# 0xPARC/plonky2-aes

Measured on AMD Instinct MI355X. Metric: proofs/sec (AES-GCM 1 KiB circuit), higher is better.
Workload: dtype u64 (Goldilocks field)

## Files before the change

### bindings/plonky2-hip/src/ffi.rs

```rust
#![allow(non_camel_case_types, dead_code)]
use std::os::raw::{c_char, c_int, c_long, c_void};

#[repr(C)] pub struct P2Builder { _private: [u8; 0] }
#[repr(C)] pub struct P2Circuit { _private: [u8; 0] }
#[repr(C)] pub struct P2Assignment { pub targets: *const u64, pub values: *const u64, pub count: usize }
#[repr(C)] #[derive(Default, Clone, Copy)]
pub struct P2CircuitInfo {
    pub degree_bits: u32, pub num_wires: u32, pub num_routed_wires: u32, pub num_constants_cols: u32, pub num_zs_cols: u32,
    pub num_quotient_cols: u32, pub num_luts: u32, pub num_ops: u32, pub num_levels: u32, pub num_slots: u32,
    pub num_virtual_targets: u32, pub num_fri_rounds: u32, pub proof_bytes: u64, pub zero_knowledge: u32, pub num_gate_kinds: u32,
    pub num_public_inputs: u32, pub hasher: u32,
}
#[repr(C)] pub struct P2KernelTime { pub name: [c_char; 48], pub ms: f32, pub count: u32 }
#[repr(C)] #[derive(Default, Clone, Copy, Debug)]
pub struct P2WitnessFault { pub kind: i32, pub op_kind: i32, pub input_index: i64, pub target: u64, pub gate_row: u32, pub computed: u64, pub found: u64 }

pub const P2_OK: c_int = 0;
pub const P2_PROOF_OK: c_int = 0;
pub const P2_VALUE_UNSET: u64 = u64::MAX;
pub const P2_FAULT_KINDS: [&str; 6] = ["NONE", "INPUT_NOT_CANONICAL", "INPUT_CONFLICT", "LOOKUP_MISS", "GENERATOR_CONFLICT", "NOT_SET"];
pub const P2_HASHER_POSEIDON: c_int = 0;
pub const P2_HASHER_KECCAK: c_int = 1;
pub const P2_POINT_WORDS: usize = 10;
pub const P2_SCALAR_LIMBS: usize = 5;
// ... 24 lines not shown
    pub fn p2_builder_split_le(a0: *mut P2Builder, x: u64, num_bits: usize, bits: *mut u64) -> c_int;
    pub fn p2_builder_range_check(a0: *mut P2Builder, x: u64, num_bits: usize) -> c_int;
    pub fn p2_builder_le_bytes_sum(a0: *mut P2Builder, bytes: *const u64, n: usize, out: *mut u64) -> c_int;
    pub fn p2_builder_split_bytes_le(a0: *mut P2Builder, x: u64, num_bytes: usize, u8_table_idx: usize, bytes: *mut u64) -> c_int;
    pub fn p2_builder_is_less_than(a0: *mut P2Builder, x: u64, y: u64, num_bits: usize, out: *mut u64) -> c_int;
    pub fn p2_builder_register_public_input(a0: *mut P2Builder, t: u64) -> c_int;
    pub fn p2_builder_add_lookup_table_from_pairs(a0: *mut P2Builder, pairs: *const u16, n_pairs: usize) -> usize;
    pub fn p2_builder_add_lookup_from_index(a0: *mut P2Builder, looking_in: u64, lut_index: usize) -> u64;
    pub fn p2_builder_num_gates(a0: *const P2Builder) -> usize;
    pub fn p2_builder_build(a0: *mut P2Builder, blob: *mut *mut u8, blob_len: *mut usize) -> c_int;
    pub fn p2_blob_free(blob: *mut u8);
    pub fn p2_aes_sbox_lut(a0: *mut P2Builder) -> usize;
    pub fn p2_aes_byte_xor_lut(a0: *mut P2Builder) -> usize;
    pub fn p2_aes_gf_2_8_mul_lut(a0: *mut P2Builder) -> usize;
    pub fn p2_gcm_u8_unit_right_shift_lut(a0: *mut P2Builder) -> usize;
    pub fn p2_gcm_u8_bitref_lut(a0: *mut P2Builder) -> usize;
    pub fn p2_gcm_clmul_lo_lut(a0: *mut P2Builder) -> usize;
    pub fn p2_gcm_clmul_hi_lut(a0: *mut P2Builder) -> usize;
    pub fn p2_aes_add_virtual_byte_target(a0: *mut P2Builder, u8_table_idx: usize) -> u64;
    pub fn p2_aes_add_virtual_byte_target_unsafe(a0: *mut P2Builder) -> u64;
    pub fn p2_aes_state_sub_bytes(a0: *mut P2Builder, sbox_lut: usize, s: *const u64, out: *mut u64);
    pub fn p2_aes_state_mix_columns(a0: *mut P2Builder, xor_lut: usize, mul_lut: usize, s: *const u64, out: *mut u64);
    pub fn p2_aes_gf_2_8_mul(a0: *mut P2Builder, mul_lut: usize, x: u64, y: u64) -> u64;
    pub fn p2_aes_gf_2_8_add(a0: *mut P2Builder, xor_lut: usize, x: u64, y: u64) -> u64;
    pub fn p2_aes_key_expansion(a0: *mut P2Builder, nk: c_int, nr: c_int, xor_lut: usize, sbox_lut: usize, key: *const u64, out: *mut u64);
    pub fn p2_aes_encrypt_block(a0: *mut P2Builder, nr: c_int, xor_lut: usize, mul_lut: usize, sbox_lut: usize, state: *const u64, expanded_key: *const u64, out_state: *mut u64);
    pub fn p2_gcm_gctr(a0: *mut P2Builder, nr: c_int, xor_lut: usize, mul_lut: usize, sbox_lut: usize, expanded_key: *const u64, icb: *const u64, x: *const u64, len: usize, y: *mut u64);
    pub fn p2_gcm_right_shift_one(a0: *mut P2Builder, shift_lut: usize, v: *const u64, out: *mut u64);
    pub fn p2_gcm_inc32(a0: *mut P2Builder, block: *const u64, out: *mut u64);
    pub fn p2_gcm_gf_2_128_mul(a0: *mut P2Builder, xor_lut: usize, shift_lut: usize, bitref_lut: usize, x: *const u64, y: *const u64, out: *mut u64);
    pub fn p2_gcm_ghash(a0: *mut P2Builder, xor_lut: usize, shift_lut: usize, bitref_lut: usize, h: *const u64, x: *const u64, len: usize, out: *mut u64) -> c_int;
    pub fn p2_gcm_gf_2_128_mul_tables(a0: *mut P2Builder, xor_lut: usize, clmul_lo_lut: usize, clmul_hi_lut: usize, x: *const u64, y: *const u64, out: *mut u64) -> c_int;
    pub fn p2_gcm_ghash_tables(a0: *mut P2Builder, xor_lut: usize, clmul_lo_lut: usize, clmul_hi_lut: usize, h: *const u64, x: *const u64, len: usize, out: *mut u64, lanes: c_int) -> c_int;
    pub fn p2_builder_set_ghash_tables(a0: *mut P2Builder, lanes: c_int) -> c_int;
    pub fn p2_aes_gcm_build(a0: *mut P2Builder, nk: c_int, nr: c_int, L: usize, with_tag: c_int, key: *mut u64, nonce: *mut u64, pt: *mut u64, ct: *mut u64, tag: *mut u64) -> c_int;
    pub fn p2_builder_hash_n_to_m_no_pad(a0: *mut P2Builder, inputs: *const u64, n: usize, outputs: *mut u64, m: usize) -> c_int;
    pub fn p2_builder_permute_swapped(a0: *mut P2Builder, inputs: *const u64, swap: u64, out: *mut u64) -> c_int;
    pub fn p2_builder_hash_or_noop(a0: *mut P2Builder, inputs: *const u64, n: usize, out: *mut u64) -> c_int;
    pub fn p2_builder_add_virtual_hash(a0: *mut P2Builder, out: *mut u64) -> c_int;
    pub fn p2_builder_add_virtual_cap(a0: *mut P2Builder, cap_height: c_int, out: *mut u64) -> c_int;
    pub fn p2_builder_connect_hashes(a0: *mut P2Builder, x: *const u64, y: *const u64) -> c_int;
    pub fn p2_builder_verify_merkle_proof_to_cap(a0: *mut P2Builder, leaf: *const u64, leaf_len: usize, index_bits: *const u64, n_bits: usize, cap: *const u64, cap_height: c_int, siblings: *const u64, n_siblings: usize) -> c_int;
    pub fn p2_builder_verify_merkle_proof(a0: *mut P2Builder, leaf: *const u64, leaf_len: usize, index_bits: *const u64, n_bits: usize, root: *const u64, siblings: *const u64, n_siblings: usize) -> c_int;
    pub fn p2_native_merkle_cap(leaves: *const u64, num_leaves: usize, leaf_len: usize, cap_height: c_int, cap: *mut u64) -> c_int;
    pub fn p2_native_merkle_prove(leaves: *const u64, num_leaves: usize, leaf_len: usize, cap_height: c_int, index: usize, siblings: *mut u64) -> c_int;
    pub fn p2_native_merkle_verify(leaf: *const u64, leaf_len: usize, index: usize, siblings: *const u64, depth: usize, cap: *const u64, cap_height: c_int, status: *mut c_int) -> c_int;
    pub fn p2_poseidon_cipher_build(a0: *mut P2Builder, L: usize, ks: *mut u64, m: *mut u64, nonce: *mut u64, ct: *mut u64) -> c_int;
    pub fn p2_native_hash_n_to_m_no_pad(in: *const u64, n: usize, out: *mut u64, m: usize);
    pub fn p2_native_poseidon_encrypt(ks10: *const u64, msg: *const u64, n_msg: usize, nonce2: *const u64, ct: *mut u64);
    pub fn p2_native_poseidon_decrypt(ks10: *const u64, ct: *const u64, n_ct: usize, nonce2: *const u64, l: usize, msg: *mut u64) -> c_int;
    pub fn p2_ecgfp5_group_order(out: *mut u64);
    pub fn p2_ecgfp5_generator(out: *mut u64);
    pub fn p2_ecgfp5_mul(k: *const u64, p: *const u64, out: *mut u64);
    pub fn p2_ecgfp5_add(p: *const u64, q: *const u64, out: *mut u64);
    pub fn p2_ecgfp5_neg(p: *const u64, out: *mut u64);
    pub fn p2_ecgfp5_is_in_subgroup(p: *const u64) -> c_int;
    pub fn p2_ecgfp5_compress(p: *const u64, w: *mut u64);
    pub fn p2_ecgfp5_decompress(w: *const u64, out: *mut u64) -> c_int;
    pub fn p2_ecgfp5_random_scalar(out: *mut u64) -> c_int;
    pub fn p2_ecgfp5_random_point(out: *mut u64) -> c_int;
    pub fn p2_ecgfp5_encode_binary(limbs: *const u32, out: *mut u64) -> c_int;
    pub fn p2_ecgfp5_random_scalar_seeded(seed: u64, out: *mut u64);
    pub fn p2_ecgfp5_random_point_seeded(seed: u64, out: *mut u64);
    pub fn p2_ecgfp5_encode_binary_seeded(limbs: *const u32, seed: u64, out: *mut u64);
    pub fn p2_ecgfp5_decode_binary(p: *const u64, limbs: *mut u32);
    pub fn p2_elgamal_encrypt(pk: *const u64, nonce: *const u64, msg: *const u64, c0: *mut u64, c1: *mut u64) -> c_int;
    pub fn p2_elgamal_decrypt(sk: *const u64, c0: *const u64, c1: *const u64, msg: *mut u64) -> c_int;
    pub fn p2_hashed_elgamal_encrypt(pk: *const u64, nonce: *const u64, msg: *const u64, c0: *mut u64, ct: *mut u64) -> c_int;
    pub fn p2_hashed_elgamal_decrypt(sk: *const u64, c0: *const u64, ct: *const u64, msg: *mut u64) -> c_int;
    pub fn p2_builder_add_virtual_point_target(a0: *mut P2Builder, out: *mut u64);
    pub fn p2_builder_constant_point(a0: *mut P2Builder, p: *const u64, out: *mut u64);
    pub fn p2_builder_add_virtual_biguint320_target(a0: *mut P2Builder, bits: *mut u64);
    pub fn p2_builder_multiply_point(a0: *mut P2Builder, bits: *const u64, p: *const u64, out: *mut u64) -> c_int;
    pub fn p2_builder_add_point(a0: *mut P2Builder, p: *const u64, q: *const u64, out: *mut u64);
    pub fn p2_builder_set_ec_gate(a0: *mut P2Builder, on: c_int) -> c_int;
    pub fn p2_builder_ec_step(a0: *mut P2Builder, acc: *const u64, q: *const u64, bit: u64, hinted: c_int, mid: *mut u64, out: *mut u64) -> c_int;
    pub fn p2_builder_public_key(a0: *mut P2Builder, sk_bits: *const u64, pk: *mut u64) -> c_int;
    pub fn p2_builder_elgamal_encrypt(a0: *mut P2Builder, pk: *const u64, nonce_bits: *const u64, msg: *const u64, c0: *mut u64, c1: *mut u64) -> c_int;
    pub fn p2_builder_hashed_elgamal_encrypt(a0: *mut P2Builder, pk: *const u64, nonce_bits: *const u64, msg: *const u64, c0: *mut u64, ct: *mut u64) -> c_int;
    pub fn p2_selftest_host(seed: u64, n_reductions: usize, n_permutations: usize) -> c_int;
    pub fn p2_selftest_device(seed: u64, threads: usize, device: c_int) -> c_int;
    pub fn p2_selftest_lazy_device(seed: u64, threads: usize, device: c_int) -> c_int;
    pub fn p2_selftest_ntt_device(seed: u64, threads: usize, device: c_int) -> c_int;
    pub fn p2_host_poseidon_known(states: *mut u64, n_perm: usize, kind: c_int, rows: u32, parts: c_int) -> c_int;
    pub fn p2_host_partial_rounds(states: *mut u64, count: usize) -> c_int;
    pub fn p2_host_merged_middle(states: *mut u64, count: usize) -> c_int;
    pub fn p2_host_ecstep_constraints(wires: *const u64, count: usize, out: *mut u64) -> c_int;
    pub fn p2_host_ecstep_constraints_ext(wires: *const u64, count: usize, out: *mut u64) -> c_int;
    pub fn p2_host_hash_leaves(data: *const u64, cols: usize, active_cols: usize, num_leaves: usize, digests: *mut u64) -> c_int;
    pub fn p2_native_gf_2_8_mul(a: u8, b: u8) -> u8;
    pub fn p2_native_aes_key_expansion(key: *const u8, nk: c_int, nr: c_int, out: *mut u8);
    pub fn p2_native_aes_encrypt_block(key: *const u8, nk: c_int, nr: c_int, in16: *const u8, out16: *mut u8);
    pub fn p2_native_gf_2_128_mul(x16: *const u8, y16: *const u8, out16: *mut u8);
    pub fn p2_native_ghash(h16: *const u8, x: *const u8, len: usize, out16: *mut u8);
    pub fn p2_native_gctr(key: *const u8, nk: c_int, nr: c_int, icb16: *const u8, x: *const u8, len: usize, y: *mut u8);
    pub fn p2_native_aes_gcm_encrypt(key: *const u8, nk: c_int, nr: c_int, nonce12: *const u8, pt: *const u8, len: usize, ct: *mut u8, tag16: *mut u8);
    pub fn p2_native_keccak_hash_no_pad(in: *const u64, n: usize, out4: *mut u64);
    pub fn p2_native_keccak_two_to_one(l4: *const u64, r4: *const u64, out4: *mut u64);
    pub fn p2_native_keccak256(data: *const u8, len: usize, out32: *mut u8);
    pub fn p2_blob_info(blob: *const u8, len: usize, out: *mut P2CircuitInfo) -> c_int;
    pub fn p2_witness_schedule_check(blob: *const u8, len: usize, fuse: u32, out: *mut u32) -> c_int;
    pub fn p2_verify(blob: *const u8, blob_len: usize, verifier_data: *const u64, verifier_data_len: usize, proof: *const u8, proof_len: usize) -> c_int;
    pub fn p2_vanishing_terms(blob: *const u8, blob_len: usize, openings: *const u8, len: usize, challenges: *const u64, pi_hash: *const u64, terms: *mut u64, cap: usize, n_terms: *mut usize, sides: *mut u64, verdict: *mut c_int) -> c_int;
    pub fn p2_proof_compress(blob: *const u8, blob_len: usize, verifier_data: *const u64, verifier_data_len: usize, proof: *const u8, proof_len: usize, out: *mut u8, cap: usize, n_written: *mut usize) -> c_int;
    pub fn p2_proof_decompress(blob: *const u8, blob_len: usize, verifier_data: *const u64, verifier_data_len: usize, cproof: *const u8, cproof_len: usize, out: *mut u8, cap: usize, n_written: *mut usize) -> c_int;
    pub fn p2_verify_compressed(blob: *const u8, blob_len: usize, verifier_data: *const u64, verifier_data_len: usize, cproof: *const u8, cproof_len: usize) -> c_int;
    pub fn p2_proof_public_inputs(blob: *const u8, blob_len: usize, proof: *const u8, proof_len: usize, out: *mut u64, cap: usize, n_written: *mut usize) -> c_int;
    pub fn p2_circuit_load(blob: *const u8, len: usize, device: c_int) -> *mut P2Circuit;
    pub fn p2_circuit_free(a0: *mut P2Circuit);
    pub fn p2_circuit_verifier_data(a0: *const P2Circuit, out: *mut u64, cap: usize, n_written: *mut usize) -> c_int;
    pub fn p2_circuit_chunk_proofs(a0: *mut P2Circuit) -> usize;
    pub fn p2_circuit_set_zk_key(a0: *mut P2Circuit, key: *const u64) -> c_int;
    pub fn p2_circuit_set_zk_seed(a0: *mut P2Circuit, seed: u64) -> c_int;
    pub fn p2_circuit_proof_bytes(a0: *const P2Circuit) -> usize;
    pub fn p2_circuit_num_public_inputs(a0: *const P2Circuit) -> usize;
    pub fn p2_circuit_public_inputs(a0: *const P2Circuit, proof: *const u8, proof_len: usize, out: *mut u64, cap: usize, n_written: *mut usize) -> c_int;
    pub fn p2_prove_batch(a0: *mut P2Circuit, batch: usize, inputs: *const P2Assignment, proofs: *mut u8, status: *mut c_int) -> c_int;
    pub fn p2_prove_batch_multi(handles: *const *mut P2Circuit, n_handles: usize, batch: usize, inputs: *const P2Assignment, proofs: *mut u8, status: *mut c_int) -> c_int;
    pub fn p2_prove_batch_device(a0: *mut P2Circuit, batch: usize, targets: *const u64, n_targets: usize, d_values: *const u64, d_proofs: *mut u8, d_status: *mut c_int, stream: *mut c_void) -> c_int;
    pub fn p2_circuit_synchronize(a0: *mut P2Circuit) -> c_int;
    pub fn p2_prove_batch_outputs_device(a0: *mut P2Circuit, batch: usize, targets: *const u64, n_targets: usize, d_values: *const u64, out_targets: *const u64, n_out: usize, d_out: *mut u64, d_proofs: *mut u8, d_status: *mut c_int, stream: *mut c_void) -> c_int;
    pub fn p2_prove_batch_outputs(a0: *mut P2Circuit, batch: usize, inputs: *const P2Assignment, out_targets: *const u64, n_out: usize, out_values: *mut u64, proofs: *mut u8, status: *mut c_int) -> c_int;
    pub fn p2_witness_batch_device(a0: *mut P2Circuit, batch: usize, targets: *const u64, n_targets: usize, d_values: *const u64, out_targets: *const u64, n_out: usize, d_out: *mut u64, d_status: *mut c_int, stream: *mut c_void) -> c_int;
    pub fn p2_witness_batch(a0: *mut P2Circuit, batch: usize, inputs: *const P2Assignment, out_targets: *const u64, n_out: usize, out_values: *mut u64, status: *mut c_int) -> c_int;
    pub fn p2_witness_explain(a0: *mut P2Circuit, input: *const P2Assignment, status: *mut c_int, out: *mut c_void) -> c_int;
    pub fn p2_host_witness(blob: *const u8, len: usize, input: *const P2Assignment, out_targets: *const u64, n_out: usize, out_values: *mut u64, status: *mut c_int, fault: *mut c_void) -> c_int;
    pub fn p2_verify_batch(a0: *mut P2Circuit, batch: usize, proofs: *const u8, verifier_data: *const u64, vd_len: usize, status: *mut c_int) -> c_int;
    pub fn p2_verify_batch_device(a0: *mut P2Circuit, batch: usize, d_proofs: *const u8, verifier_data: *const u64, vd_len: usize, d_status: *mut c_int, stream: *mut c_void) -> c_int;
    pub fn p2_gpu_vanishing_flags(a0: *mut P2Circuit, batch: usize, buffers: *const u8, challenges: *const u64, pi_hashes: *const u64, flags: *mut u32) -> c_int;
    pub fn p2_compress_batch(a0: *mut P2Circuit, batch: usize, proofs: *const u8, verifier_data: *const u64, vd_len: usize, out: *mut u8, lengths: *mut u32, status: *mut c_int) -> c_int;
    pub fn p2_decompress_batch(a0: *mut P2Circuit, batch: usize, cproofs: *const u8, lengths: *const u32, verifier_data: *const u64, vd_len: usize, out: *mut u8, status: *mut c_int) -> c_int;
    pub fn p2_verify_compressed_batch(a0: *mut P2Circuit, batch: usize, cproofs: *const u8, lengths: *const u32, verifier_data: *const u64, vd_len: usize, status: *mut c_int) -> c_int;
    pub fn p2_compress_batch_device(a0: *mut P2Circuit, batch: usize, d_proofs: *const u8, verifier_data: *const u64, vd_len: usize, d_out: *mut u8, d_lengths: *mut u32, d_status: *mut c_int, stream: *mut c_void) -> c_int;
    pub fn p2_decompress_batch_device(a0: *mut P2Circuit, batch: usize, d_cproofs: *const u8, d_lengths: *const u32, verifier_data: *const u64, vd_len: usize, d_out: *mut u8, d_status: *mut c_int, stream: *mut c_void) -> c_int;
    pub fn p2_verify_compressed_batch_device(a0: *mut P2Circuit, batch: usize, d_cproofs: *const u8, d_lengths: *const u32, verifier_data: *const u64, vd_len: usize, d_status: *mut c_int, stream: *mut c_void) -> c_int;
    pub fn p2_circuit_set_option(a0: *mut P2Circuit, name: *const c_char, value: c_long) -> c_int;
    pub fn p2_circuit_set_timing(a0: *mut P2Circuit, enable: c_int) -> c_int;
    pub fn p2_circuit_get_timing(a0: *mut P2Circuit, out: *mut P2KernelTime, cap: usize) -> usize;
    pub fn p2_merkle_tree_new(leaves: *const u64, num_leaves: usize, leaf_len: usize, cap_height: c_int, device: c_int, tree: *mut *mut c_void) -> c_int;
    pub fn p2_merkle_tree_new_device(d_leaves: *const u64, num_leaves: usize, leaf_len: usize, cap_height: c_int, device: c_int, stream: *mut c_void, tree: *mut *mut c_void) -> c_int;
    pub fn p2_merkle_tree_free(tree: *mut c_void);
    pub fn p2_merkle_tree_cap(tree: *mut c_void, cap: *mut u64, cap_words: usize) -> c_int;
    pub fn p2_merkle_tree_prove_batch(tree: *mut c_void, indices: *const u64, n: usize, siblings: *mut u64) -> c_int;
    pub fn p2_merkle_tree_prove_batch_device(tree: *mut c_void, d_indices: *const u64, n: usize, d_out: *mut u64, out_stride_words: usize, d_status: *mut c_int, stream: *mut c_void) -> c_int;
    pub fn p2_merkle_verify_batch(leaves: *const u64, leaf_len: usize, indices: *const u64, siblings: *const u64, depth: usize, cap: *const u64, cap_height: c_int, n: usize, status: *mut c_int, device: c_int) -> c_int;
    pub fn p2_merkle_verify_batch_device(d_leaves: *const u64, leaf_len: usize, d_indices: *const u64, d_siblings: *const u64, depth: usize, d_cap: *const u64, cap_height: c_int, n: usize, d_status: *mut c_int, device: c_int, stream: *mut c_void) -> c_int;
    pub fn p2_gpu_merkle_build_device(d_leaves: *const u64, num_leaves: usize, leaf_len: usize, cap_height: c_int, with_transpose: c_int, d_scratch: *mut u64, d_dig: *mut u64, device: c_int, stream: *mut c_void) -> c_int;
    pub fn p2_gpu_device_count() -> c_int;
    pub fn p2_gpu_poseidon(states: *mut u64, n_perm: usize, device: c_int) -> c_int;
    pub fn p2_gpu_lde(coeffs: *const u64, cols: usize, degree_bits: c_int, rate_bits: c_int, lde: *mut u64, device: c_int) -> c_int;
    pub fn p2_gpu_intt(values: *const u64, cols: usize, degree_bits: c_int, coeffs: *mut u64, device: c_int) -> c_int;
    pub fn p2_gpu_lde_round(coeffs: *const u64, cols: usize, degree_bits: c_int, arities: *const u32, n_rounds: usize, round: usize, batch: usize, in_batch_stride: usize, out: *mut u64, out_batch_stride: usize, device: c_int) -> c_int;
    pub fn p2_gpu_quotient_chunks(qvals: *const u64, chunks: usize, degree_bits: c_int, batch: usize, out: *mut u64, device: c_int) -> c_int;
    pub fn p2_gpu_merkle_cap(cols_major: *const u64, cols: usize, num_leaves: usize, cap_height: c_int, cap: *mut u64, device: c_int) -> c_int;
    pub fn p2_gpu_merkle_cap_hasher(cols_major: *const u64, cols: usize, num_leaves: usize, cap_height: c_int, hasher: c_int, cap: *mut u64, device: c_int) -> c_int;
    pub fn p2_gpu_hash_leaves(data: *const u64, cols: usize, active_cols: usize, num_leaves: usize, batch: usize, digests: *mut u64, device: c_int) -> c_int;
    pub fn p2_gpu_partial_rounds(states: *mut u64, count: usize, device: c_int) -> c_int;
    pub fn p2_gpu_merged_middle(states: *mut u64, count: usize, device: c_int) -> c_int;
    pub fn p2_gpu_ecstep_constraints(wires: *const u64, count: usize, out: *mut u64, device: c_int) -> c_int;
    pub fn p2_gpu_merkle_level(child: *const u64, num_parents: usize, batch: usize, parent: *mut u64, device: c_int) -> c_int;
    pub fn p2_gpu_hash_fri_leaves(vals: *const u64, len: usize, arity: c_int, batch: usize, digests: *mut u64, device: c_int) -> c_int;
    pub fn p2_gpu_zeta_pows(z: *const u64, n: usize, pows: *mut u64, device: c_int) -> c_int;
    pub fn p2_circuit_debug_read(a0: *mut P2Circuit, name: *const c_char, index: usize, out: *mut u64, cap: usize, n_written: *mut usize) -> c_int;
}
```

### include/p2aes.h

```cpp
#ifndef P2AES_H
#define P2AES_H
#include <stddef.h>
#include <stdint.h>

#ifdef __cplusplus
extern "C" {
#endif

enum {
    P2_OK = 0,
    P2_ERR_INVALID = 1,
    P2_ERR_NO_DEVICE = 2,
    P2_ERR_HIP = 3,
    P2_ERR_VERIFY = 4
};
enum {
    P2_PROOF_OK = 0,
    P2_PROOF_WITNESS_CONFLICT = 1,
    P2_PROOF_MISSING_INPUT = 2,
    P2_PROOF_ZETA_IN_SUBGROUP = 3,
    P2_PROOF_POW_NOT_FOUND = 4
};
enum {
    P2_VERIFY_OK = 0,
// ... 55 lines not shown
p2_target p2_aes_add_virtual_byte_target(p2_builder*, size_t u8_table_idx);
p2_target p2_aes_add_virtual_byte_target_unsafe(p2_builder*);
void p2_aes_state_sub_bytes(p2_builder*, size_t sbox_lut, const p2_target* s, p2_target* out);
void p2_aes_state_mix_columns(p2_builder*, size_t xor_lut, size_t mul_lut, const p2_target* s, p2_target* out);
p2_target p2_aes_gf_2_8_mul(p2_builder*, size_t mul_lut, p2_target x, p2_target y);
p2_target p2_aes_gf_2_8_add(p2_builder*, size_t xor_lut, p2_target x, p2_target y);
void p2_aes_key_expansion(p2_builder*, int nk, int nr, size_t xor_lut, size_t sbox_lut, const p2_target* key, p2_target* out);
void p2_aes_encrypt_block(p2_builder*, int nr, size_t xor_lut, size_t mul_lut, size_t sbox_lut, const p2_target* state,
                          const p2_target* expanded_key, p2_target* out_state);
void p2_gcm_gctr(p2_builder*, int nr, size_t xor_lut, size_t mul_lut, size_t sbox_lut, const p2_target* expanded_key,
                 const p2_target* icb, const p2_target* x, size_t len, p2_target* y);
void p2_gcm_right_shift_one(p2_builder*, size_t shift_lut, const p2_target* v, p2_target* out);
void p2_gcm_inc32(p2_builder*, const p2_target* block, p2_target* out);
void p2_gcm_gf_2_128_mul(p2_builder*, size_t xor_lut, size_t shift_lut, size_t bitref_lut, const p2_target* x,
                         const p2_target* y, p2_target* out);
int p2_gcm_ghash(p2_builder*, size_t xor_lut, size_t shift_lut, size_t bitref_lut, const p2_target* h, const p2_target* x,
                 size_t len, p2_target* out);
int p2_gcm_gf_2_128_mul_tables(p2_builder*, size_t xor_lut, size_t clmul_lo_lut, size_t clmul_hi_lut, const p2_target* x,
                               const p2_target* y, p2_target* out);
int p2_gcm_ghash_tables(p2_builder*, size_t xor_lut, size_t clmul_lo_lut, size_t clmul_hi_lut, const p2_target* h,
                        const p2_target* x, size_t len, p2_target* out, int lanes);
int p2_builder_set_ghash_tables(p2_builder*, int lanes);
int p2_aes_gcm_build(p2_builder*, int nk, int nr, size_t L, int with_tag, p2_target* key, p2_target* nonce, p2_target* pt,
                     p2_target* ct, p2_target* tag);

int p2_builder_hash_n_to_m_no_pad(p2_builder*, const p2_target* inputs, size_t n, p2_target* outputs, size_t m);
int p2_builder_permute_swapped(p2_builder*, const p2_target inputs[12], p2_target swap, p2_target out[12]);
int p2_builder_hash_or_noop(p2_builder*, const p2_target* inputs, size_t n, p2_target out[4]);
int p2_builder_add_virtual_hash(p2_builder*, p2_target out[4]);
int p2_builder_add_virtual_cap(p2_builder*, int cap_height, p2_target* out);
int p2_builder_connect_hashes(p2_builder*, const p2_target x[4], const p2_target y[4]);
int p2_builder_verify_merkle_proof_to_cap(p2_builder*, const p2_target* leaf, size_t leaf_len, const p2_target* index_bits, size_t n_bits,
                                          const p2_target* cap, int cap_height, const p2_target* siblings, size_t n_siblings);
int p2_builder_verify_merkle_proof(p2_builder*, const p2_target* leaf, size_t leaf_len, const p2_target* index_bits, size_t n_bits,
                                   const p2_target root[4], const p2_target* siblings, size_t n_siblings);
int p2_native_merkle_cap(const uint64_t* leaves, size_t num_leaves, size_t leaf_len, int cap_height, uint64_t* cap);
int p2_native_merkle_prove(const uint64_t* leaves, size_t num_leaves, size_t leaf_len, int cap_height, size_t index, uint64_t* siblings);
int p2_native_merkle_verify(const uint64_t* leaf, size_t leaf_len, size_t index, const uint64_t* siblings, size_t depth, const uint64_t* cap,
                            int cap_height, int* status);
int p2_poseidon_cipher_build(p2_builder*, size_t L, p2_target* ks, p2_target* m, p2_target* nonce, p2_target* ct);
void p2_native_hash_n_to_m_no_pad(const uint64_t* in, size_t n, uint64_t* out, size_t m);
void p2_native_poseidon_encrypt(const uint64_t* ks10, const uint64_t* msg, size_t n_msg, const uint64_t* nonce2, uint64_t* ct);
int p2_native_poseidon_decrypt(const uint64_t* ks10, const uint64_t* ct, size_t n_ct, const uint64_t* nonce2, size_t l, uint64_t* msg);

#define P2_POINT_WORDS 10
#define P2_SCALAR_LIMBS 5
#define P2_SCALAR_BITS 320
void p2_ecgfp5_group_order(uint64_t out[5]);
void p2_ecgfp5_generator(uint64_t out[10]);
void p2_ecgfp5_mul(const uint64_t k[5], const uint64_t p[10], uint64_t out[10]);
void p2_ecgfp5_add(const uint64_t p[10], const uint64_t q[10], uint64_t out[10]);
void p2_ecgfp5_neg(const uint64_t p[10], uint64_t out[10]);
int p2_ecgfp5_is_in_subgroup(const uint64_t p[10]);
void p2_ecgfp5_compress(const uint64_t p[10], uint64_t w[5]);
int p2_ecgfp5_decompress(const uint64_t w[5], uint64_t out[10]);
int p2_ecgfp5_random_scalar(uint64_t out[5]);
int p2_ecgfp5_random_point(uint64_t out[10]);
int p2_ecgfp5_encode_binary(const uint32_t limbs[5], uint64_t out[10]);
void p2_ecgfp5_random_scalar_seeded(uint64_t seed, uint64_t out[5]);
void p2_ecgfp5_random_point_seeded(uint64_t seed, uint64_t out[10]);
void p2_ecgfp5_encode_binary_seeded(const uint32_t limbs[5], uint64_t seed, uint64_t out[10]);
void p2_ecgfp5_decode_binary(const uint64_t p[10], uint32_t limbs[5]);
int p2_elgamal_encrypt(const uint64_t pk[10], const uint64_t nonce[5], const uint64_t msg[10], uint64_t c0[10], uint64_t c1[10]);
int p2_elgamal_decrypt(const uint64_t sk[5], const uint64_t c0[10], const uint64_t c1[10], uint64_t msg[10]);
int p2_hashed_elgamal_encrypt(const uint64_t pk[10], const uint64_t nonce[5], const uint64_t msg[5], uint64_t c0[10], uint64_t ct[5]);
int p2_hashed_elgamal_decrypt(const uint64_t sk[5], const uint64_t c0[10], const uint64_t ct[5], uint64_t msg[5]);
void p2_builder_add_virtual_point_target(p2_builder*, p2_target out[10]);
void p2_builder_constant_point(p2_builder*, const uint64_t p[10], p2_target out[10]);
void p2_builder_add_virtual_biguint320_target(p2_builder*, p2_target bits[320]);
int p2_builder_multiply_point(p2_builder*, const p2_target bits[320], const p2_target p[10], p2_target out[10]);
void p2_builder_add_point(p2_builder*, const p2_target p[10], const p2_target q[10], p2_target out[10]);
int p2_builder_set_ec_gate(p2_builder*, int on);
int p2_builder_ec_step(p2_builder*, const p2_target acc[20], const p2_target q[10], p2_target bit, int hinted, p2_target mid[20], p2_target out[20]);
int p2_builder_public_key(p2_builder*, const p2_target sk_bits[320], p2_target pk[10]);
int p2_builder_elgamal_encrypt(p2_builder*, const p2_target pk[10], const p2_target nonce_bits[320], const p2_target msg[10],
                               p2_target c0[10], p2_target c1[10]);
int p2_builder_hashed_elgamal_encrypt(p2_builder*, const p2_target pk[10], const p2_target nonce_bits[320], const p2_target msg[5],
                                      p2_target c0[10], p2_target ct[5]);

int p2_selftest_host(uint64_t seed, size_t n_reductions, size_t n_permutations);
int p2_selftest_device(uint64_t seed, size_t threads, int device);
int p2_selftest_lazy_device(uint64_t seed, size_t threads, int device);
int p2_selftest_ntt_device(uint64_t seed, size_t threads, int device);
int p2_host_poseidon_known(uint64_t* states, size_t n_perm, int kind, uint32_t rows, int parts);
int p2_host_partial_rounds(uint64_t* states, size_t count);
int p2_host_merged_middle(uint64_t* states, size_t count);
int p2_host_ecstep_constraints(const uint64_t* wires, size_t count, uint64_t* out);
int p2_host_ecstep_constraints_ext(const uint64_t* wires, size_t count, uint64_t* out);
int p2_host_hash_leaves(const uint64_t* data, size_t cols, size_t active_cols, size_t num_leaves, uint64_t* digests);

uint8_t p2_native_gf_2_8_mul(uint8_t a, uint8_t b);
void p2_native_aes_key_expansion(const uint8_t* key, int nk, int nr, uint8_t* out );
void p2_native_aes_encrypt_block(const uint8_t* key, int nk, int nr, const uint8_t* in16, uint8_t* out16);
void p2_native_gf_2_128_mul(const uint8_t* x16, const uint8_t* y16, uint8_t* out16);
void p2_native_ghash(const uint8_t* h16, const uint8_t* x, size_t len, uint8_t* out16);
void p2_native_gctr(const uint8_t* key, int nk, int nr, const uint8_t* icb16, const uint8_t* x, size_t len, uint8_t* y);
void p2_native_aes_gcm_encrypt(const uint8_t* key, int nk, int nr, const uint8_t* nonce12, const uint8_t* pt, size_t len,
                               uint8_t* ct, uint8_t* tag16);

void p2_native_keccak_hash_no_pad(const uint64_t* in, size_t n, uint64_t out4[4]);
void p2_native_keccak_two_to_one(const uint64_t l4[4], const uint64_t r4[4], uint64_t out4[4]);
void p2_native_keccak256(const uint8_t* data, size_t len, uint8_t out32[32]);

typedef struct {
    uint32_t degree_bits, num_wires, num_routed_wires, num_constants_cols, num_zs_cols, num_quotient_cols, num_luts,
        num_ops, num_levels, num_slots, num_virtual_targets, num_fri_rounds;
    uint64_t proof_bytes;
    uint32_t zero_knowledge, num_gate_kinds;
    uint32_t num_public_inputs;
    uint32_t hasher;
} p2_circuit_info;
int p2_blob_info(const uint8_t* blob, size_t len, p2_circuit_info* out);
int p2_witness_schedule_check(const uint8_t* blob, size_t len, uint32_t fuse, uint32_t out[4]);
int p2_verify(const uint8_t* blob, size_t blob_len, const uint64_t* verifier_data, size_t verifier_data_len,
              const uint8_t* proof, size_t proof_len);
int p2_vanishing_terms(const uint8_t* blob, size_t blob_len, const uint8_t* openings, size_t len, const uint64_t challenges[16],
                       const uint64_t pi_hash[4], uint64_t* terms, size_t cap, size_t* n_terms, uint64_t sides[8], int* verdict);
int p2_proof_compress(const uint8_t* blob, size_t blob_len, const uint64_t* verifier_data, size_t verifier_data_len, const uint8_t* proof,
                      size_t proof_len, uint8_t* out, size_t cap, size_t* n_written);
int p2_proof_decompress(const uint8_t* blob, size_t blob_len, const uint64_t* verifier_data, size_t verifier_data_len, const uint8_t* cproof,
                        size_t cproof_len, uint8_t* out, size_t cap, size_t* n_written);
int p2_verify_compressed(const uint8_t* blob, size_t blob_len, const uint64_t* verifier_data, size_t verifier_data_len,
                         const uint8_t* cproof, size_t cproof_len);
int p2_proof_public_inputs(const uint8_t* blob, size_t blob_len, const uint8_t* proof, size_t proof_len, uint64_t* out, size_t cap,
                           size_t* n_written);

typedef struct p2_circuit p2_circuit;
p2_circuit* p2_circuit_load(const uint8_t* blob, size_t len, int device);
void p2_circuit_free(p2_circuit*);
int p2_circuit_verifier_data(const p2_circuit*, uint64_t* out, size_t cap, size_t* n_written);
size_t p2_circuit_chunk_proofs(p2_circuit*);
int p2_circuit_set_zk_key(p2_circuit*, const uint64_t key[4]);
int p2_circuit_set_zk_seed(p2_circuit*, uint64_t seed);
size_t p2_circuit_proof_bytes(const p2_circuit*);
size_t p2_circuit_num_public_inputs(const p2_circuit*);
int p2_circuit_public_inputs(const p2_circuit*, const uint8_t* proof, size_t proof_len, uint64_t* out, size_t cap, size_t* n_written);
typedef struct {
    const p2_target* targets;
    const uint64_t* values;
    size_t count;
} p2_assignment;
int p2_prove_batch(p2_circuit*, size_t batch, const p2_assignment* inputs, uint8_t* proofs, int* status);
int p2_prove_batch_multi(p2_circuit* const* handles, size_t n_handles, size_t batch, const p2_assignment* inputs,
                         uint8_t* proofs, int* status);
int p2_prove_batch_device(p2_circuit*, size_t batch, const p2_target* targets, size_t n_targets, const uint64_t* d_values,
                          uint8_t* d_proofs, int* d_status, void* stream);
int p2_circuit_synchronize(p2_circuit*);

#define P2_VALUE_UNSET UINT64_MAX
int p2_prove_batch_outputs_device(p2_circuit*, size_t batch, const p2_target* targets, size_t n_targets, const uint64_t* d_values,
                                  const p2_target* out_targets, size_t n_out, uint64_t* d_out, uint8_t* d_proofs, int* d_status, void* stream);
int p2_prove_batch_outputs(p2_circuit*, size_t batch, const p2_assignment* inputs, const p2_target* out_targets, size_t n_out,
                           uint64_t* out_values, uint8_t* proofs, int* status);
int p2_witness_batch_device(p2_circuit*, size_t batch, const p2_target* targets, size_t n_targets, const uint64_t* d_values,
                            const p2_target* out_targets, size_t n_out, uint64_t* d_out, int* d_status, void* stream);
int p2_witness_batch(p2_circuit*, size_t batch, const p2_assignment* inputs, const p2_target* out_targets, size_t n_out,
                     uint64_t* out_values, int* status);
typedef struct {
    int32_t kind;
    int32_t op_kind;
    int64_t input_index;
    p2_target target;
    uint32_t gate_row;
    uint64_t computed, found;
} p2_witness_fault;
enum {
// ... 75 lines not shown
```

### plonky2-aes_amd/api.py

```python
import ctypes as C
import os
import struct

P = 0xFFFFFFFF00000001


class P2Error(RuntimeError):
    pass


class ProveError(P2Error):

    def __init__(self, status):
        self.status = status
        super().__init__({1: "witness conflict or lookup input not in table", 2: "a generator never ran (missing input)",
                          3: "opening point is in the subgroup",
                          4: "no proof-of-work witness found"}.get(status, "prove failed (%d)" % status))


VERIFY_OK, VERIFY_SHAPE, VERIFY_NON_CANONICAL, VERIFY_POW, VERIFY_ZETA_IN_SUBGROUP, VERIFY_VANISHING = 0, 1, 2, 3, 4, 5
VERIFY_MERKLE_INITIAL, VERIFY_FRI_FOLD, VERIFY_MERKLE_FRI, VERIFY_FINAL_POLY = 6, 7, 8, 9
VERIFY_REASONS = {
    "": VERIFY_OK,
    "proof truncated": VERIFY_SHAPE,
# ... 106 lines not shown
    _fields_ = [("name", C.c_char * 48), ("ms", C.c_float), ("count", C.c_uint32)]


def lib():
    global _lib
    if _lib is not None:
        return _lib
    path = lib_path()
    if not os.path.exists(path):
        raise P2Error("native library %s is missing: run `python -c 'import __graft_entry__ as g; g.build()'`" % path)
    L = C.CDLL(path)
    vp = C.c_void_p
    sig = {
        "p2_last_error": (C.c_char_p, []),
        "p2_builder_new": (vp, []), "p2_builder_new_zk": (vp, []), "p2_builder_free": (None, [vp]),
        "p2_builder_new_config": (vp, [C.c_int, C.c_int]), "p2_builder_set_hasher": (C.c_int, [vp, C.c_int]),
        "p2_native_keccak_hash_no_pad": (None, [u64p, sz, u64p]), "p2_native_keccak_two_to_one": (None, [u64p, u64p, u64p]),
        "p2_native_keccak256": (None, [C.c_char_p, sz, C.c_char_p]),
        "p2_gpu_merkle_cap_hasher": (C.c_int, [u64p, sz, sz, C.c_int, C.c_int, u64p, C.c_int]),
        "p2_circuit_set_zk_seed": (C.c_int, [vp, u64]),
        "p2_circuit_set_zk_key": (C.c_int, [vp, C.POINTER(u64)]),
        "p2_circuit_set_option": (C.c_int, [vp, C.c_char_p, C.c_long]),
        "p2_prove_batch_multi": (C.c_int, [C.POINTER(vp), sz, sz, C.POINTER(_Assignment), C.c_char_p, C.POINTER(C.c_int)]),
        "p2_builder_add_virtual_target": (u64, [vp]), "p2_builder_constant": (u64, [vp, u64]),
        "p2_builder_zero": (u64, [vp]), "p2_builder_one": (u64, [vp]),
        "p2_builder_arithmetic": (u64, [vp, u64, u64, u64, u64, u64]),
        "p2_builder_mul_const_add": (u64, [vp, u64, u64, u64]),
        "p2_builder_add": (u64, [vp, u64, u64]), "p2_builder_sub": (u64, [vp, u64, u64]), "p2_builder_mul": (u64, [vp, u64, u64]),
        "p2_builder_select": (u64, [vp, u64, u64, u64]), "p2_builder_is_equal": (u64, [vp, u64, u64]),
        "p2_builder_connect": (None, [vp, u64, u64]),
        "p2_builder_assert_bool": (C.c_int, [vp, u64]), "p2_builder_range_check": (C.c_int, [vp, u64, sz]),
        "p2_builder_le_sum": (C.c_int, [vp, u64p, sz, u64p]), "p2_builder_le_bytes_sum": (C.c_int, [vp, u64p, sz, u64p]),
        "p2_builder_split_le": (C.c_int, [vp, u64, sz, u64p]), "p2_builder_split_bytes_le": (C.c_int, [vp, u64, sz, sz, u64p]),
        "p2_builder_is_less_than": (C.c_int, [vp, u64, u64, sz, u64p]),
        "p2_builder_register_public_input": (C.c_int, [vp, u64]),
        "p2_proof_public_inputs": (C.c_int, [C.c_char_p, sz, C.c_char_p, sz, u64p, sz, C.POINTER(sz)]),
        "p2_builder_add_lookup_table_from_pairs": (sz, [vp, u16p, sz]),
        "p2_builder_add_lookup_from_index": (u64, [vp, u64, sz]),
        "p2_builder_num_gates": (sz, [vp]),
        "p2_builder_build": (C.c_int, [vp, C.POINTER(u8p), C.POINTER(sz)]), "p2_blob_free": (None, [u8p]),
        "p2_aes_sbox_lut": (sz, [vp]), "p2_aes_byte_xor_lut": (sz, [vp]), "p2_aes_gf_2_8_mul_lut": (sz, [vp]),
        "p2_gcm_u8_unit_right_shift_lut": (sz, [vp]), "p2_gcm_u8_bitref_lut": (sz, [vp]),
        "p2_aes_add_virtual_byte_target": (u64, [vp, sz]), "p2_aes_add_virtual_byte_target_unsafe": (u64, [vp]),
        "p2_aes_state_sub_bytes": (None, [vp, sz, u64p, u64p]),
        "p2_aes_state_mix_columns": (None, [vp, sz, sz, u64p, u64p]),
        "p2_aes_gf_2_8_mul": (u64, [vp, sz, u64, u64]), "p2_aes_gf_2_8_add": (u64, [vp, sz, u64, u64]),
        "p2_aes_key_expansion": (None, [vp, C.c_int, C.c_int, sz, sz, u64p, u64p]),
        "p2_aes_encrypt_block": (None, [vp, C.c_int, sz, sz, sz, u64p, u64p, u64p]),
        "p2_gcm_gctr": (None, [vp, C.c_int, sz, sz, sz, u64p, u64p, u64p, sz, u64p]),
        "p2_gcm_right_shift_one": (None, [vp, sz, u64p, u64p]), "p2_gcm_inc32": (None, [vp, u64p, u64p]),
        "p2_gcm_gf_2_128_mul": (None, [vp, sz, sz, sz, u64p, u64p, u64p]),
        "p2_gcm_ghash": (C.c_int, [vp, sz, sz, sz, u64p, u64p, sz, u64p]),
        "p2_gcm_clmul_lo_lut": (sz, [vp]), "p2_gcm_clmul_hi_lut": (sz, [vp]),
        "p2_gcm_gf_2_128_mul_tables": (C.c_int, [vp, sz, sz, sz, u64p, u64p, u64p]),
        "p2_gcm_ghash_tables": (C.c_int, [vp, sz, sz, sz, u64p, u64p, sz, u64p, C.c_int]),
        "p2_builder_set_ghash_tables": (C.c_int, [vp, C.c_int]),
        "p2_aes_gcm_build": (C.c_int, [vp, C.c_int, C.c_int, sz, C.c_int, u64p, u64p, u64p, u64p, u64p]),
        "p2_builder_hash_n_to_m_no_pad": (C.c_int, [vp, u64p, sz, u64p, sz]),
        "p2_poseidon_cipher_build": (C.c_int, [vp, sz, u64p, u64p, u64p, u64p]),
        "p2_native_hash_n_to_m_no_pad": (None, [u64p, sz, u64p, sz]),
        "p2_native_poseidon_encrypt": (None, [u64p, u64p, sz, u64p, u64p]),
        "p2_native_poseidon_decrypt": (C.c_int, [u64p, u64p, sz, u64p, sz, u64p]),
        "p2_ecgfp5_group_order": (None, [u64p]), "p2_ecgfp5_generator": (None, [u64p]),
        "p2_ecgfp5_mul": (None, [u64p, u64p, u64p]), "p2_ecgfp5_add": (None, [u64p, u64p, u64p]), "p2_ecgfp5_neg": (None, [u64p, u64p]),
        "p2_ecgfp5_is_in_subgroup": (C.c_int, [u64p]),
        "p2_ecgfp5_compress": (None, [u64p, u64p]), "p2_ecgfp5_decompress": (C.c_int, [u64p, u64p]),
        "p2_ecgfp5_random_scalar": (C.c_int, [u64p]), "p2_ecgfp5_random_point": (C.c_int, [u64p]),
        "p2_ecgfp5_encode_binary": (C.c_int, [u32p, u64p]),
        "p2_ecgfp5_random_scalar_seeded": (None, [u64, u64p]), "p2_ecgfp5_random_point_seeded": (None, [u64, u64p]),
        "p2_ecgfp5_encode_binary_seeded": (None, [u32p, u64, u64p]), "p2_ecgfp5_decode_binary": (None, [u64p, u32p]),
        "p2_elgamal_encrypt": (C.c_int, [u64p, u64p, u64p, u64p, u64p]), "p2_elgamal_decrypt": (C.c_int, [u64p, u64p, u64p, u64p]),
        "p2_hashed_elgamal_encrypt": (C.c_int, [u64p, u64p, u64p, u64p, u64p]),
        "p2_hashed_elgamal_decrypt": (C.c_int, [u64p, u64p, u64p, u64p]),
        "p2_builder_add_virtual_point_target": (None, [vp, u64p]), "p2_builder_constant_point": (None, [vp, u64p, u64p]),
        "p2_builder_add_virtual_biguint320_target": (None, [vp, u64p]),
        "p2_builder_multiply_point": (C.c_int, [vp, u64p, u64p, u64p]), "p2_builder_add_point": (None, [vp, u64p, u64p, u64p]),
        "p2_builder_public_key": (C.c_int, [vp, u64p, u64p]),
        "p2_builder_set_ec_gate": (C.c_int, [vp, C.c_int]), "p2_builder_ec_step": (C.c_int, [vp, u64p, u64p, u64, C.c_int, u64p, u64p]),
        "p2_builder_elgamal_encrypt": (C.c_int, [vp, u64p, u64p, u64p, u64p, u64p]),
        "p2_builder_hashed_elgamal_encrypt": (C.c_int, [vp, u64p, u64p, u64p, u64p, u64p]),
        "p2_selftest_host": (C.c_int, [u64, sz, sz]), "p2_selftest_device": (C.c_int, [u64, sz, C.c_int]),
        "p2_selftest_lazy_device": (C.c_int, [u64, sz, C.c_int]),
        "p2_selftest_ntt_device": (C.c_int, [u64, sz, C.c_int]),
        "p2_native_gf_2_8_mul": (C.c_uint8, [C.c_uint8, C.c_uint8]),
        "p2_native_aes_key_expansion": (None, [C.c_char_p, C.c_int, C.c_int, C.c_char_p]),
        "p2_native_aes_encrypt_block": (None, [C.c_char_p, C.c_int, C.c_int, C.c_char_p, C.c_char_p]),
        "p2_native_gf_2_128_mul": (None, [C.c_char_p, C.c_char_p, C.c_char_p]),
        "p2_native_ghash": (None, [C.c_char_p, C.c_char_p, sz, C.c_char_p]),
        "p2_native_gctr": (None, [C.c_char_p, C.c_int, C.c_int, C.c_char_p, C.c_char_p, sz, C.c_char_p]),
        "p2_native_aes_gcm_encrypt": (None, [C.c_char_p, C.c_int, C.c_int, C.c_char_p, C.c_char_p, sz, C.c_char_p, C.c_char_p]),
        "p2_blob_info": (C.c_int, [C.c_char_p, sz, C.POINTER(_Info)]),
        "p2_witness_schedule_check": (C.c_int, [C.c_char_p, sz, C.c_uint32, u32p]),
        "p2_verify": (C.c_int, [C.c_char_p, sz, u64p, sz, C.c_char_p, sz]),
        "p2_vanishing_terms": (C.c_int, [C.c_char_p, sz, C.c_char_p, sz, u64p, u64p, u64p, sz, C.POINTER(sz), u64p, C.POINTER(C.c_int)]),
        "p2_gpu_vanishing_flags": (C.c_int, [vp, sz, C.c_char_p, u64p, u64p, u32p]),
        "p2_proof_compress": (C.c_int, [C.c_char_p, sz, u64p, sz, C.c_char_p, sz, C.c_char_p, sz, C.POINTER(sz)]),
        "p2_proof_decompress": (C.c_int, [C.c_char_p, sz, u64p, sz, C.c_char_p, sz, C.c_char_p, sz, C.POINTER(sz)]),
        "p2_verify_compressed": (C.c_int, [C.c_char_p, sz, u64p, sz, C.c_char_p, sz]),
        "p2_circuit_load": (vp, [C.c_char_p, sz, C.c_int]), "p2_circuit_free": (None, [vp]),
        "p2_circuit_verifier_data": (C.c_int, [vp, u64p, sz, C.POINTER(sz)]),
        "p2_circuit_proof_bytes": (sz, [vp]),
        "p2_circuit_num_public_inputs": (sz, [vp]),
        "p2_circuit_public_inputs": (C.c_int, [vp, C.c_char_p, sz, u64p, sz, C.POINTER(sz)]),
        "p2_circuit_chunk_proofs": (sz, [vp]),
        "p2_prove_batch": (C.c_int, [vp, sz, C.POINTER(_Assignment), C.c_char_p, C.POINTER(C.c_int)]),
        "p2_prove_batch_device": (C.c_int, [vp, sz, u64p, sz, vp, vp, vp, vp]),
        "p2_circuit_synchronize": (C.c_int, [vp]),
        "p2_prove_batch_outputs": (C.c_int, [vp, sz, C.POINTER(_Assignment), u64p, sz, u64p, C.c_char_p, C.POINTER(C.c_int)]),
        "p2_prove_batch_outputs_device": (C.c_int, [vp, sz, u64p, sz, vp, u64p, sz, vp, vp, vp, vp]),
        "p2_witness_batch": (C.c_int, [vp, sz, C.POINTER(_Assignment), u64p, sz, u64p, C.POINTER(C.c_int)]),
        "p2_witness_batch_device": (C.c_int, [vp, sz, u64p, sz, vp, u64p, sz, vp, vp, vp]),
        "p2_witness_explain": (C.c_int, [vp, C.POINTER(_Assignment), C.POINTER(C.c_int), vp]),
        "p2_host_witness": (C.c_int, [C.c_char_p, sz, C.POINTER(_Assignment), u64p, sz, u64p, C.POINTER(C.c_int), vp]),
        "p2_verify_batch": (C.c_int, [vp, sz, C.c_char_p, u64p, sz, C.POINTER(C.c_int)]),
        "p2_verify_batch_device": (C.c_int, [vp, sz, vp, u64p, sz, vp, vp]),
        "p2_compress_batch": (C.c_int, [vp, sz, C.c_char_p, u64p, sz, C.c_char_p, u32p, C.POINTER(C.c_int)]),
        "p2_compress_batch_device": (C.c_int, [vp, sz, vp, u64p, sz, vp, vp, vp, vp]),
        "p2_decompress_batch": (C.c_int, [vp, sz, C.c_char_p, u32p, u64p, sz, C.c_char_p, C.POINTER(C.c_int)]),
        "p2_decompress_batch_device": (C.c_int, [vp, sz, vp, vp, u64p, sz, vp, vp, vp]),
        "p2_verify_compressed_batch": (C.c_int, [vp, sz, C.c_char_p, u32p, u64p, sz, C.POINTER(C.c_int)]),
        "p2_verify_compressed_batch_device": (C.c_int, [vp, sz, vp, vp, u64p, sz, vp, vp]),
        "p2_circuit_set_timing": (C.c_int, [vp, C.c_int]),
        "p2_circuit_get_timing": (sz, [vp, C.POINTER(_KernelTime), sz]),
        "p2_gpu_device_count": (C.c_int, []),
        "p2_gpu_poseidon": (C.c_int, [u64p, sz, C.c_int]),
        "p2_host_partial_rounds": (C.c_int, [u64p, sz]),
        "p2_gpu_partial_rounds": (C.c_int, [u64p, sz, C.c_int]),
        "p2_host_merged_middle": (C.c_int, [u64p, sz]),
        "p2_gpu_merged_middle": (C.c_int, [u64p, sz, C.c_int]),
        "p2_host_ecstep_constraints": (C.c_int, [u64p, sz, u64p]), "p2_host_ecstep_constraints_ext": (C.c_int, [u64p, sz, u64p]),
        "p2_gpu_ecstep_constraints": (C.c_int, [u64p, sz, u64p, C.c_int]),
        "p2_gpu_lde": (C.c_int, [u64p, sz, C.c_int, C.c_int, u64p, C.c_int]),
        "p2_gpu_intt": (C.c_int, [u64p, sz, C.c_int, u64p, C.c_int]),
        "p2_gpu_lde_round": (C.c_int, [u64p, sz, C.c_int, u32p, sz, sz, sz, sz, u64p, sz, C.c_int]),
        "p2_gpu_quotient_chunks": (C.c_int, [u64p, sz, C.c_int, sz, u64p, C.c_int]),
        "p2_gpu_merkle_cap": (C.c_int, [u64p, sz, sz, C.c_int, u64p, C.c_int]),
        "p2_gpu_zeta_pows": (C.c_int, [u64p, sz, u64p, C.c_int]),
        "p2_circuit_debug_read": (C.c_int, [vp, C.c_char_p, sz, u64p, sz, C.POINTER(sz)]),
        "p2_builder_permute_swapped": (C.c_int, [vp, u64p, u64, u64p]), "p2_builder_hash_or_noop": (C.c_int, [vp, u64p, sz, u64p]),
        "p2_builder_add_virtual_hash": (C.c_int, [vp, u64p]), "p2_builder_add_virtual_cap": (C.c_int, [vp, C.c_int, u64p]),
        "p2_builder_connect_hashes": (C.c_int, [vp, u64p, u64p]),
        "p2_builder_verify_merkle_proof_to_cap": (C.c_int, [vp, u64p, sz, u64p, sz, u64p, C.c_int, u64p, sz]),
        "p2_builder_verify_merkle_proof": (C.c_int, [vp, u64p, sz, u64p, sz, u64p, u64p, sz]),
        "p2_native_merkle_cap": (C.c_int, [u64p, sz, sz, C.c_int, u64p]),
        "p2_native_merkle_prove": (C.c_int, [u64p, sz, sz, C.c_int, sz, u64p]),
        "p2_native_merkle_verify": (C.c_int, [u64p, sz, sz, u64p, sz, u64p, C.c_int, C.POINTER(C.c_int)]),
        "p2_merkle_tree_new": (C.c_int, [u64p, sz, sz, C.c_int, C.c_int, C.POINTER(vp)]),
        "p2_merkle_tree_new_device": (C.c_int, [vp, sz, sz, C.c_int, C.c_int, vp, C.POINTER(vp)]),
        "p2_merkle_tree_free": (None, [vp]), "p2_merkle_tree_cap": (C.c_int, [vp, u64p, sz]),
        "p2_merkle_tree_prove_batch": (C.c_int, [vp, u64p, sz, u64p]),
        "p2_merkle_tree_prove_batch_device": (C.c_int, [vp, vp, sz, vp, sz, vp, vp]),
        "p2_merkle_verify_batch": (C.c_int, [u64p, sz, u64p, u64p, sz, u64p, C.c_int, sz, C.POINTER(C.c_int), C.c_int]),
        "p2_merkle_verify_batch_device": (C.c_int, [vp, sz, vp, vp, sz, vp, C.c_int, sz, vp, C.c_int, vp]),
        "p2_gpu_merkle_build_device": (C.c_int, [vp, sz, sz, C.c_int, C.c_int, vp, vp, C.c_int, vp]),
    }
    missing = []
    for name, (res, args) in sig.items():
        try:
            f = getattr(L, name)
        except AttributeError:
            missing.append(name)
            continue
        f.restype, f.argtypes = res, args
    L._p2_missing = missing
    L._p2_signatures = sig
    _lib = L
# ... 1047 lines not shown
```

### plonky2-aes_amd/csrc/capi_host.cpp

```cpp
#include <stdlib.h>

#include "../../include/p2aes.h"
#include "aes_gadgets.h"
#include "capi_common.h"
#include "compress.h"
#include "ecgfp5.h"
#include "merkle_host.h"
#include "poseidon_cipher.h"
#include "poseidon_fast.h"
#include "verifier.h"
#include "witness_check.h"
#include "witness_schedule.h"

using namespace p2;

namespace p2 {
thread_local std::string g_last_error;
}

struct p2_builder {
    CircuitBuilder b;
};


// ... 531 lines not shown
        ptt_put(ecgfp5::multiply_point(b->b, bits_at(bits), ptt_at(p)), out);
        return P2_OK;
    } catch (std::exception& e) {
        return set_error(e.what()), P2_ERR_INVALID;
    }
}
void p2_builder_add_point(p2_builder* b, const p2_target p[10], const p2_target q[10], p2_target out[10]) { (void)guarded([&] {    ptt_put(ecgfp5::add_point(b->b, ptt_at(p), ptt_at(q)), out);}); }
int p2_builder_public_key(p2_builder* b, const p2_target sk_bits[320], p2_target pk[10]) {
    try {
        ptt_put(ecgfp5::public_key_target(b->b, bits_at(sk_bits)), pk);
        return P2_OK;
    } catch (std::exception& e) {
        return set_error(e.what()), P2_ERR_INVALID;
    }
}
int p2_builder_elgamal_encrypt(p2_builder* b, const p2_target pk[10], const p2_target nonce_bits[320], const p2_target msg[10], p2_target c0[10],
                               p2_target c1[10]) {
    try {
        ecgfp5::PointTarget a, c;
        ecgfp5::elgamal_encrypt_target(b->b, ptt_at(pk), bits_at(nonce_bits), ptt_at(msg), &a, &c);
        ptt_put(a, c0);
        ptt_put(c, c1);
        return P2_OK;
    } catch (std::exception& e) {
        return set_error(e.what()), P2_ERR_INVALID;
    }
}
int p2_builder_hashed_elgamal_encrypt(p2_builder* b, const p2_target pk[10], const p2_target nonce_bits[320], const p2_target msg[5],
                                      p2_target c0[10], p2_target ct[5]) {
    try {
        ecgfp5::PointTarget a;
        ecgfp5::hashed_elgamal_encrypt_target(b->b, ptt_at(pk), bits_at(nonce_bits), msg, &a, ct);
        ptt_put(a, c0);
        return P2_OK;
    } catch (std::exception& e) {
        return set_error(e.what()), P2_ERR_INVALID;
    }
}

int p2_selftest_host(uint64_t seed, size_t n_reductions, size_t n_permutations) {
    u64 x = seed | 1;
    auto rnd = [&]() {
        x ^= x << 13;
        x ^= x >> 7;
        x ^= x << 17;
        return x;
    };
    size_t bad = 0;
    for (size_t i = 0; i < n_reductions; i++) {
        u64 hi = rnd(), lo = rnd();
        switch (i & 15) {
            case 0: hi &= gl::EPS; break;
            case 1: lo &= gl::EPS; break;
            case 2: hi |= ~gl::EPS; break;
            case 3: lo |= ~gl::EPS; break;
            case 4: hi = 0; break;
            case 5: lo = 0; break;
            case 6: hi = ~0ull; lo = ~0ull - (x & 3); break;
            case 7: hi &= ~gl::EPS; lo &= gl::EPS; break;
            default: break;
        }
        unsigned __int128 v = ((unsigned __int128)hi << 64) | lo;
        u64 want = (u64)(v % gl::P);
        if (glf::canon(glf::red128(hi, lo)) != want) bad++;
        if (gl::reduce128(hi, lo) != want) bad++;
        glf::Acc a;
        a.init();
        a.fma(hi, lo);
        a.fma(lo, lo);
        unsigned __int128 w = ((unsigned __int128)hi * lo) % gl::P + ((unsigned __int128)lo * lo) % gl::P;
        if (glf::canon(a.reduce()) != (u64)(w % gl::P)) bad++;
    }
    for (size_t i = 0; i < n_permutations; i++) {
        u64 s0[12], s1[12];
        for (int k = 0; k < 12; k++) s0[k] = s1[k] = (i & 3) == 3 ? rnd() : rnd() % gl::P;
        for (int k = 0; k < 12; k++) s0[k] %= gl::P;
        gl::poseidon(s0);
        glf::poseidon(s1);
        for (int k = 0; k < 12; k++) bad += s0[k] != s1[k];
    }
    return (int)std::min<size_t>(bad, 0x7FFFFFFF);
}

int p2_host_poseidon_known(uint64_t* states, size_t n_perm, int kind, uint32_t rows, int parts) {
    if (kind < 0 || kind > (int)glf::FR_ZERO_RATE || rows == 0 || rows > glf::ROWS_ALL) return set_error("kind must be 0..2 and rows a mask of words 0..11"), P2_ERR_INVALID;
    for (size_t i = 0; i < n_perm; i++) {
        u64* s = states + 12 * i;
        if (parts) {
            glf::first_round_any(s, (u32)kind);
            glf::middle(s);
            glf::last_round_any(s, rows);
        } else {
            glf::permute_known_any(s, (u32)kind, rows);
        }
    }
    return P2_OK;
}
int p2_host_partial_rounds(uint64_t* states, size_t count) {
    for (size_t i = 0; i < count; i++) glf::partial_block(states + 12 * i);
    return P2_OK;
}
int p2_host_merged_middle(uint64_t* states, size_t count) {
    for (size_t i = 0; i < count; i++) glf::merged_middle(states + 12 * i);
    return P2_OK;
}
int p2_host_ecstep_constraints(const uint64_t* wires, size_t count, uint64_t* out) {
    if (count && (!wires || !out)) return set_error("p2_host_ecstep_constraints: null argument"), P2_ERR_INVALID;
    for (size_t i = 0; i < 80 * count; i++)
        if (wires[i] >= gl::P) return set_error("p2_host_ecstep_constraints: non-canonical wire"), P2_ERR_INVALID;
    for (size_t r = 0; r < count; r++)
        ecstep_gate_constraints<FBase>([&](u32 i) { return wires[80 * r + i]; }, [&](int k, u64 c) { out[40 * r + k] = c; });
    return P2_OK;
}
int p2_host_ecstep_constraints_ext(const uint64_t* wires, size_t count, uint64_t* out) {
    if (count && (!wires || !out)) return set_error("p2_host_ecstep_constraints_ext: null argument"), P2_ERR_INVALID;
    for (size_t i = 0; i < 160 * count; i++)
        if (wires[i] >= gl::P) return set_error("p2_host_ecstep_constraints_ext: non-canonical wire"), P2_ERR_INVALID;
    for (size_t r = 0; r < count; r++)
        ecstep_gate_constraints<FExt>([&](u32 i) { return gl::e2(wires[160 * r + 2 * i], wires[160 * r + 2 * i + 1]); },
                                      [&](int k, gl::E2 c) { out[80 * r + 2 * k] = c.a, out[80 * r + 2 * k + 1] = c.b; });
    return P2_OK;
}
int p2_host_hash_leaves(const uint64_t* data, size_t cols, size_t active_cols, size_t num_leaves, uint64_t* digests) {
    if (cols == 0 || cols > (1u << 20)) return set_error("cols out of range"), P2_ERR_INVALID;
    for (size_t leaf = 0; leaf < num_leaves; leaf++) {
        u64 st[12] = {0};
        u64* out = digests + 4 * leaf;
        if (cols <= 4) {
            for (size_t c = 0; c < 4; c++) out[c] = (c < cols && c < active_cols) ? data[c * num_leaves + leaf] : 0;
            continue;
        }
        for (size_t c0 = 0; c0 < cols; c0 += 8) {
            for (size_t k = 0; k < 8 && c0 + k < cols; k++) st[k] = c0 + k < active_cols ? data[(c0 + k) * num_leaves + leaf] : 0;
            glf::sponge_permute(st, (int)c0, (int)cols, (int)std::min(active_cols, cols));
        }
        for (int i = 0; i < 4; i++) out[i] = st[i];
    }
    return P2_OK;
}

uint8_t p2_native_gf_2_8_mul(uint8_t a, uint8_t b) { return aes::gf_2_8_mul(a, b); }
void p2_native_aes_key_expansion(const uint8_t* key, int nk, int nr, uint8_t* out) {
    (void)guarded([&] {
        auto w = aes::key_expansion(nk, nr, key);
        for (size_t i = 0; i < w.size(); i++) memcpy(out + 4 * i, w[i].data(), 4);
    });
}
void p2_native_aes_encrypt_block(const uint8_t* key, int nk, int nr, const uint8_t* in, uint8_t* out) {
    (void)guarded([&] {
        auto w = aes::key_expansion(nk, nr, key);
        auto s = aes::flatten_state(aes::encrypt_block(nr, in, w));
        memcpy(out, s.data(), 16);
    });
}
void p2_native_gf_2_128_mul(const uint8_t* x, const uint8_t* y, uint8_t* out) {
    (void)guarded([&] {
        auto r = aes::gf_2_128_mul(x, y);
        memcpy(out, r.data(), 16);
    });
}
void p2_native_ghash(const uint8_t* h, const uint8_t* x, size_t len, uint8_t* out) {
    (void)guarded([&] {
        auto r = aes::ghash(h, x, len);
        memcpy(out, r.data(), 16);
    });
}
// ... 331 lines not shown
```

### plonky2-aes_amd/csrc/gl.h

```cpp
#pragma once
#include <stdint.h>

#if defined(__HIPCC__)
#include <hip/hip_runtime.h>
#define GL_HD __host__ __device__ __forceinline__
#define GL_D __device__ __forceinline__
#else
#define GL_HD inline
#define GL_D inline
#endif

namespace gl {

typedef uint64_t u64;
typedef uint32_t u32;

static const u64 P = 0xFFFFFFFF00000001ULL;
static const u64 EPS = 0xFFFFFFFFULL;
static const u64 MULT_GEN = 14293326489335486720ULL;
static const u64 POW2_GEN = 7277203076849721926ULL;
static const u64 W_EXT = 7;

#if defined(__HIP_DEVICE_COMPILE__)
typedef unsigned long long sg;
// ... 22 lines not shown
    sg dead;
    asm("v_mad_u64_u32 %0, %1, %2, %3, %4" : "=v"(r), "=s"(dead) : "v"(x), "n"(K), "s"(acc_uniform));
    return r;
}
template <u32 K>
GL_D u64 madk0(u32 x) {
    static_assert(K <= 64, "not an inline constant");
    u64 r;
    sg dead;
    asm("v_mad_u64_u32 %0, %1, %2, %3, 0" : "=v"(r), "=s"(dead) : "v"(x), "n"(K));
    return r;
}
GL_D u64 mad_eps_co(u32 a, u64 c, sg& k) {
    u64 r;
    asm("v_mad_u64_u32 %0, %1, %2, -1, %3" : "=v"(r), "=s"(k) : "v"(a), "v"(c));
    return r;
}
GL_D u64 add_u32(u64 c, u32 x) {
    u64 r;
    sg dead;
    asm("v_mad_u64_u32 %0, %1, %2, 1, %3" : "=v"(r), "=s"(dead) : "v"(x), "v"(c));
    return r;
}
GL_D u64 add_eps_co(u64 c, sg& k) {
    u64 r;
    asm("v_mad_u64_u32 %0, %1, 1, -1, %2" : "=v"(r), "=s"(k) : "v"(c));
    return r;
}
GL_D u32 add_co(u32 x, u32 y, sg& cout) {
    u32 r;
    asm("v_add_co_u32_e64 %0, %1, %2, %3" : "=v"(r), "=s"(cout) : "v"(x), "v"(y));
    return r;
}
GL_D u32 addc_co(u32 x, u32 y, sg cin, sg& cout) {
    u32 r;
    asm("s_nop 1\n\tv_addc_co_u32_e64 %0, %1, %2, %3, %4" : "=v"(r), "=s"(cout) : "v"(x), "v"(y), "s"(cin));
    return r;
}
GL_D u32 sub_co(u32 x, u32 y, sg& cout) {
    u32 r;
    asm("v_sub_co_u32_e64 %0, %1, %2, %3" : "=v"(r), "=s"(cout) : "v"(x), "v"(y));
    return r;
}
GL_D u32 subb_co(u32 x, u32 y, sg cin, sg& cout) {
    u32 r;
    asm("s_nop 1\n\tv_subb_co_u32_e64 %0, %1, %2, %3, %4" : "=v"(r), "=s"(cout) : "v"(x), "v"(y), "s"(cin));
    return r;
}
GL_D u32 subb_co_settled(u32 x, u32 y, sg cin, sg& cout) {
    u32 r;
    asm("v_subb_co_u32_e64 %0, %1, %2, %3, %4" : "=v"(r), "=s"(cout) : "v"(x), "v"(y), "s"(cin));
    return r;
}
GL_D u64 add_eps_where_settled(sg C, u64 Rs) {
    u64 out;
    u32 c01;
    sg dead;
    asm("v_cndmask_b32_e64 %[c], 0, 1, %[m]\n\t"
        "v_mad_u64_u32 %[o], %[d], %[c], -1, %[r]"
        : [o] "=&v"(out), [c] "=&v"(c01), [d] "=&s"(dead)
        : [m] "s"(C), [r] "v"(Rs));
    return out;
}
GL_D u32 subb0_co(u32 x, sg cin, sg& cout) {
    u32 r;
    asm("s_nop 1\n\tv_subb_co_u32_e64 %0, %1, %2, 0, %3" : "=v"(r), "=s"(cout) : "v"(x), "s"(cin));
    return r;
}
GL_D u32 ones_where(sg m) {
    u32 r;
    asm("s_nop 1\n\tv_cndmask_b32_e64 %0, 0, -1, %1" : "=v"(r) : "s"(m));
    return r;
}
GL_D u32 pick(sg m, u32 yes, u32 no) {
    u32 r;
    asm("s_nop 1\n\tv_cndmask_b32_e64 %0, %1, %2, %3" : "=v"(r) : "v"(no), "v"(yes), "s"(m));
    return r;
}
GL_D u32 one_where(sg m) {
    u32 r;
    asm("s_nop 1\n\tv_cndmask_b32_e64 %0, 0, 1, %1" : "=v"(r) : "s"(m));
    return r;
}
template <bool BRANCH = true>
GL_D u64 red_fix(u64 Rs, sg C, sg B) {
    if (!BRANCH) {
        const u32 dh = ones_where(B & ~C);
        const u32 dl = ones_where(C & ~B) - dh;
        u64 d = ((u64)dh << 32) | dl;
        asm("" : "+v"(d));
        return Rs + d;
    }
    sg Cm = C;
    if (__builtin_expect(B != 0, 0)) {
        const u32 dh = ones_where(B & ~C);
        u64 d = ((u64)dh << 32) | (0u - dh);
        asm("" : "+v"(d));
        Rs += d;
        Cm = C & ~B;
    }
    return add_eps_where_settled(Cm, Rs);
}
GL_D u64 pick64(sg m, u64 yes, u64 no) {
    u32 lo, hi;
    asm("s_nop 1\n\tv_cndmask_b32_e64 %0, %3, %2, %6\n\tv_cndmask_b32_e64 %1, %5, %4, %6"
        : "=&v"(lo), "=&v"(hi)
        : "v"((u32)yes), "v"((u32)no), "v"((u32)(yes >> 32)), "v"((u32)(no >> 32)), "s"(m));
    return ((u64)hi << 32) | lo;
}
GL_D u64 pick64_salu(sg m, u64 yes, u64 no) {
    u32 lo, hi;
    asm("v_cndmask_b32_e64 %0, %3, %2, %6\n\tv_cndmask_b32_e64 %1, %5, %4, %6"
        : "=&v"(lo), "=&v"(hi)
        : "v"((u32)yes), "v"((u32)no), "v"((u32)(yes >> 32)), "v"((u32)(no >> 32)), "s"(m));
    return ((u64)hi << 32) | lo;
}
template <bool HAS_ADDEND, bool A_UNIFORM = false, bool BRANCH = true>
GL_D u64 mulr_add_dev(u64 a, u64 b, u64 c) {
    const u32 a0 = (u32)a, a1 = (u32)(a >> 32), b0 = (u32)b, b1 = (u32)(b >> 32);
    const u64 P = HAS_ADDEND ? (u64)a0 * b0 + (u32)c : (u64)a0 * b0;
    u64 Y = (u64)a0 * b1 + (P >> 32);
    if (HAS_ADDEND) Y = add_u32(Y, (u32)(c >> 32));
    sg k, C, b1_, B;
    Y = A_UNIFORM ? mad_co_k(a1, b0, Y, k) : mad_co(a1, b0, Y, k);
    const u64 H = (u64)a1 * b1 + (Y >> 32);
    const u64 lo = (Y << 32) | (u32)P;
    const u64 R = mad_eps_co((u32)H, lo, C);
    const u32 r0 = subb_co_settled((u32)R, (u32)(H >> 32), k, b1_);
    const u32 r1 = subb0_co((u32)(R >> 32), b1_, B);
    return red_fix<BRANCH>(((u64)r1 << 32) | r0, C, B);
}
GL_D u64 red128_dev(u64 hi, u64 lo) {
    sg C, b1_, B;
    const u64 R = mad_eps_co((u32)hi, lo, C);
    const u32 r0 = sub_co((u32)R, (u32)(hi >> 32), b1_);
    const u32 r1 = subb0_co((u32)(R >> 32), b1_, B);
    return red_fix(((u64)r1 << 32) | r0, C, B);
}
GL_D u64 canon_dev(u64 r) {
    sg c;
    const u64 t = add_eps_co(r, c);
    return pick64(c, t, r);
}
#endif

GL_HD u64 add(u64 a, u64 b) {
#if defined(__HIP_DEVICE_COMPILE__)
    sg k, c1, c2;
    const u32 s0 = add_co((u32)a, (u32)b, k);
    const u32 s1 = addc_co((u32)(a >> 32), (u32)(b >> 32), k, c1);
    const u64 t = add_eps_co(((u64)s1 << 32) | s0, c2);
    const sg m = c1 | c2;
    return pick64_salu(m, t, ((u64)s1 << 32) | s0);
#else
    u64 s = a + b;
    if (s < a || s >= P) s -= P;
    return s;
#endif
}
GL_HD u64 add_ref(u64 a, u64 b) {
    u64 s = a + b;
    if (s < a || s >= P) s -= P;
    return s;
}
GL_HD u64 sub(u64 a, u64 b) {
#if defined(__HIP_DEVICE_COMPILE__)
    sg b0, B;
    const u32 d0 = sub_co((u32)a, (u32)b, b0);
    const u32 d1 = subb_co((u32)(a >> 32), (u32)(b >> 32), b0, B);
    const u32 e = ones_where(B);
    u64 fix = ((u64)e << 32) | (0u - e);
    asm("" : "+v"(fix));
    return (((u64)d1 << 32) | d0) + fix;
#else
    return a >= b ? a - b : a + (P - b);
#endif
}
GL_HD u64 sub_ref(u64 a, u64 b) { return a >= b ? a - b : a + (P - b); }
GL_HD u64 neg(u64 a) { return a ? P - a : 0; }
GL_HD u64 dbl(u64 a) { return add(a, a); }

GL_HD void mul64(u64 a, u64 b, u64& hi, u64& lo) {
#if defined(__HIP_DEVICE_COMPILE__)
    lo = a * b;
    hi = __umul64hi(a, b);
#else
    unsigned __int128 m = (unsigned __int128)a * b;
    lo = (u64)m;
    hi = (u64)(m >> 64);
#endif
}

GL_HD u64 reduce128(u64 hi, u64 lo) {
    u64 hi_hi = hi >> 32, hi_lo = hi & EPS;
    u64 t0 = lo - hi_hi;
    if (lo < hi_hi) t0 -= EPS;
    u64 t1 = hi_lo * EPS;
    u64 r = t0 + t1;
    if (r < t1) r += EPS;
    if (r >= P) r -= P;
    return r;
}
GL_HD u64 mul_ref(u64 a, u64 b) {
    u64 hi, lo;
    mul64(a, b, hi, lo);
    return reduce128(hi, lo);
}
GL_HD u64 mul(u64 a, u64 b) {
#if defined(__HIP_DEVICE_COMPILE__)
    return canon_dev(mulr_add_dev<false>(a, b, 0));
#else
    return mul_ref(a, b);
#endif
}
GL_HD u64 mul_nb(u64 a, u64 b) {
#if defined(__HIP_DEVICE_COMPILE__)
    return canon_dev(mulr_add_dev<false, false, false>(a, b, 0));
#else
    return mul_ref(a, b);
#endif
}
GL_HD u64 sqr(u64 a) { return mul(a, a); }
GL_HD u64 mul_add(u64 a, u64 b, u64 c) {
#if defined(__HIP_DEVICE_COMPILE__)
    return canon_dev(mulr_add_dev<true>(a, b, c));
#else
    return add(mul(a, b), c);
#endif
}

GL_HD u64 mul_add_nc(u64 a, u64 b, u64 c) {
#if defined(__HIP_DEVICE_COMPILE__)
    return mulr_add_dev<true>(a, b, c);
#else
    return add(mul(a, b), c);
#endif
}
GL_HD u64 mul_nc(u64 a, u64 b) {
#if defined(__HIP_DEVICE_COMPILE__)
    return mulr_add_dev<false>(a, b, 0);
#else
    return mul(a, b);
#endif
}
GL_HD u64 mul_add_nc_k(u64 k, u64 b, u64 c) {
#if defined(__HIP_DEVICE_COMPILE__)
    return mulr_add_dev<true, true>(k, b, c);
#else
    return add(mul(k, b), c);
#endif
}
GL_HD u64 mul_nc_k(u64 k, u64 b) {
#if defined(__HIP_DEVICE_COMPILE__)
    return mulr_add_dev<false, true>(k, b, 0);
#else
    return mul(k, b);
#endif
}

GL_HD u64 pow(u64 b, u64 e) {
    u64 r = 1;
    while (e) {
        if (e & 1) r = mul(r, b);
        b = sqr(b);
        e >>= 1;
    }
    return r;
}
GL_HD u64 exp_pow2(u64 b, int k) {
    for (int i = 0; i < k; i++) b = sqr(b);
    return b;
}
GL_HD u64 inv(u64 a) { return pow(a, P - 2); }

GL_HD u64 root_of_unity(int k) { return exp_pow2(POW2_GEN, 32 - k); }

GL_HD u32 bitrev(u32 x, int bits) {
    u32 r = 0;
    for (int i = 0; i < bits; i++) {
        r = (r << 1) | (x & 1);
        x >>= 1;
    }
    return r;
}

struct E2 {
    u64 a, b;
};
GL_HD E2 e2(u64 a, u64 b = 0) {
    E2 r;
    r.a = a;
    r.b = b;
    return r;
}
GL_HD E2 add(E2 x, E2 y) { return e2(add(x.a, y.a), add(x.b, y.b)); }
GL_HD E2 sub(E2 x, E2 y) { return e2(sub(x.a, y.a), sub(x.b, y.b)); }
GL_HD E2 mul(E2 x, E2 y) {
    u64 a0b0 = mul(x.a, y.a), a1b1 = mul(x.b, y.b);
    u64 c0 = add(a0b0, mul(a1b1, W_EXT));
    u64 c1 = add(mul(x.a, y.b), mul(x.b, y.a));
    return e2(c0, c1);
}
GL_HD E2 mul(E2 x, u64 s) { return e2(mul(x.a, s), mul(x.b, s)); }
GL_HD E2 sqr(E2 x) { return mul(x, x); }
// ... 103 lines not shown
```

### plonky2-aes_amd/csrc/kernels.h

```cpp
#pragma once
#include <hip/hip_runtime.h>

#include "circuit.h"
#include "witness_schedule.h"
#include "gl.h"
#include "poseidon_fast.h"
#include "poseidon_gate.h"
#include "ecstep_gate.h"
#include "zk_prf.h"

namespace p2k {
using gl::E2;
using gl::u32;
using gl::u64;

static const u64 UNSET = ~0ull;

#ifndef P2_HASH_WAVES_PER_EU
#define P2_HASH_WAVES_PER_EU 5
#endif
#define P2_HASH_WAVES __attribute__((amdgpu_waves_per_eu(P2_HASH_WAVES_PER_EU, P2_HASH_WAVES_PER_EU)))

__global__ __launch_bounds__(256) P2_HASH_WAVES void k_hash_leaves(const u64* __restrict__ data, int cols, int active_cols, size_t col_stride,
                                                      size_t batch_stride, size_t num_leaves, u64* __restrict__ digests,
                                                      size_t dig_batch_stride) {
    if ((size_t)blockIdx.x * blockDim.x + threadIdx.x >= num_leaves) return;
    const u64* d = data + (size_t)blockIdx.y * batch_stride + ((size_t)blockIdx.x * blockDim.x + threadIdx.x);
    u64 st[12];
#pragma unroll
    for (int i = 0; i < 12; i++) st[i] = 0;
    if (cols <= 4) {
        u64* out = digests + (size_t)blockIdx.y * dig_batch_stride + ((size_t)blockIdx.x * blockDim.x + threadIdx.x) * 4;
        for (int c = 0; c < 4; c++) out[c] = (c < cols && c < active_cols) ? d[(size_t)c * col_stride] : 0;
        return;
    }
    for (int c0 = 0; c0 < cols; c0 += 8) {
#pragma unroll
        for (int k = 0; k < 8; k++) {
            int c = c0 + k;
            if (c < cols) st[k] = c < active_cols ? d[(size_t)k * col_stride] : 0;
        }
        d += 8 * col_stride;
        glf::sponge_permute(st, c0, cols, active_cols);
    }
    u64* out = digests + (size_t)blockIdx.y * dig_batch_stride + ((size_t)blockIdx.x * blockDim.x + threadIdx.x) * 4;
#pragma unroll
    for (int i = 0; i < 4; i++) out[i] = st[i];
}

__global__ __launch_bounds__(256) P2_HASH_WAVES void k_hash_fri_leaves(const u64* __restrict__ vals, size_t len, size_t batch_stride, int arity,
                                                          u64* __restrict__ digests, size_t dig_batch_stride) {
    size_t leaf = (size_t)blockIdx.x * blockDim.x + threadIdx.x;
    size_t num_leaves = len / arity;
    if (leaf >= num_leaves) return;
    const u64* v = vals + (size_t)blockIdx.y * batch_stride;
    u64 st[12];
#pragma unroll
    for (int i = 0; i < 12; i++) st[i] = 0;
    int width = 2 * arity;
    for (int e0 = 0; e0 < width; e0 += 8) {
#pragma unroll
        for (int k = 0; k < 8; k++) {
            int e = e0 + k;
            if (e < width) st[k] = v[(size_t)(e & 1) * len + leaf * arity + (e >> 1)];
        }
        glf::sponge_permute(st, e0, width, width);
    }
    u64* out = digests + (size_t)blockIdx.y * dig_batch_stride + leaf * 4;
#pragma unroll
    for (int i = 0; i < 4; i++) out[i] = st[i];
}

__global__ __launch_bounds__(256) P2_HASH_WAVES void k_merkle_level(const u64* __restrict__ child, u64* __restrict__ parent, size_t num_parents,
                                                       size_t batch_stride) {
    if ((size_t)blockIdx.x * blockDim.x + threadIdx.x >= num_parents) return;
    u64 st[12];
    {
        const u64* c = child + (size_t)blockIdx.y * batch_stride + 8 * ((size_t)blockIdx.x * blockDim.x + threadIdx.x);
#pragma unroll
        for (int k = 0; k < 8; k++) st[k] = c[k];
    }
#pragma unroll
    for (int k = 8; k < 12; k++) st[k] = 0;
    glf::two_to_one_permute(st);
    u64* o = parent + (size_t)blockIdx.y * batch_stride + 4 * ((size_t)blockIdx.x * blockDim.x + threadIdx.x);
#pragma unroll
    for (int k = 0; k < 4; k++) o[k] = st[k];
}

__global__ __launch_bounds__(256) P2_HASH_WAVES void k_merkle_top(u64* __restrict__ dig, size_t batch_stride, u32 bits, u32 first_level, u32 num_levels) {
    u64* base = dig + (size_t)blockIdx.y * batch_stride;
    u32 P = ((1u << bits) >> (first_level + 1)) / gridDim.x;
    for (u32 k = 0, l = first_level; k < num_levels; k++, l++, P >>= 1) {
        if (threadIdx.x < P) {
            const size_t off_c = 4 * (((size_t)2 << bits) - ((size_t)2 << (bits - l))), off_p = 4 * (((size_t)2 << bits) - ((size_t)2 << (bits - l - 1)));
            const size_t idx = (size_t)blockIdx.x * P + threadIdx.x;
            u64 st[12];
            {
                const u64* c = base + off_c + 8 * idx;
#pragma unroll
                for (int q = 0; q < 8; q++) st[q] = c[q];
            }
#pragma unroll
            for (int q = 8; q < 12; q++) st[q] = 0;
            glf::two_to_one_permute(st);
            u64* o = base + off_p + 4 * idx;
#pragma unroll
            for (int q = 0; q < 4; q++) o[q] = st[q];
        }
        __syncthreads();
    }
}
__global__ __launch_bounds__(256) void k_merkle_top_coop(u64* __restrict__ dig, size_t batch_stride, u32 bits, u32 first_level, u32 num_levels) {
    u64* base = dig + (size_t)blockIdx.y * batch_stride;
    u32 P = ((1u << bits) >> (first_level + 1)) / gridDim.x;
    const u32 g = threadIdx.x >> 4, i = threadIdx.x & 15;
    for (u32 k = 0, l = first_level; k < num_levels; k++, l++, P >>= 1) {
        const size_t off_c = 4 * (((size_t)2 << bits) - ((size_t)2 << (bits - l))), off_p = 4 * (((size_t)2 << bits) - ((size_t)2 << (bits - l - 1)));
        for (u32 first = 0; first < P; first += blockDim.x >> 4) {
            if (first + ((threadIdx.x >> 6) << 2) < P) {
                const u32 idx = first + g;
                const bool live = idx < P;
                const size_t node = (size_t)blockIdx.x * P + (live ? idx : 0);
                u64 w = (live && i < 8) ? base[off_c + 8 * node + i] : 0;
                w = glf::poseidon_coop(w, i);
                if (live && i < 4) base[off_p + 4 * node + i] = w;
            }
        }
        __syncthreads();
    }
}

__global__ void k_poseidon_states(u64* states, size_t n) {
    size_t i = (size_t)blockIdx.x * blockDim.x + threadIdx.x;
    if (i >= n) return;
    u64 st[12];
    for (int k = 0; k < 12; k++) st[k] = states[12 * i + k];
    glf::poseidon(st);
    for (int k = 0; k < 12; k++) states[12 * i + k] = st[k];
}

__global__ __launch_bounds__(256) P2_HASH_WAVES void k_partial_rounds(u64* states, size_t n) {
    size_t i = (size_t)blockIdx.x * blockDim.x + threadIdx.x;
    if (i >= n) return;
    u64 st[12];
    for (int k = 0; k < 12; k++) st[k] = states[12 * i + k];
    glf::partial_block(st);
    for (int k = 0; k < 12; k++) states[12 * i + k] = st[k];
}

__global__ __launch_bounds__(256) P2_HASH_WAVES void k_merged_middle(u64* states, size_t n) {
    size_t i = (size_t)blockIdx.x * blockDim.x + threadIdx.x;
    if (i >= n) return;
    u64 st[12];
    for (int k = 0; k < 12; k++) st[k] = states[12 * i + k];
    glf::merged_middle(st);
    for (int k = 0; k < 12; k++) states[12 * i + k] = st[k];
}

struct NttArgs {
    const u64* in;
    u64* out;
    const u64* tw;
    const u64* pre;
    const u64* pre_tw;
    const u64* post;
    u64 post_scalar;
    size_t in_col_stride, out_col_stride, in_batch_stride, out_batch_stride;
    int logn, log_nmax, cosets;
    int bitrev_in, bitrev_out;
    int in_coset_blocks;
    u32 block_of_coset[8];
};

__global__ __launch_bounds__(1024) void k_ntt_lds(NttArgs a) {
    extern __shared__ __align__(16) u64 lds[];
    const int logn = a.logn;
    const u32 n = 1u << logn;
    const u32 col = blockIdx.x / a.cosets, coset = blockIdx.x % a.cosets;
    const u32 blk = a.block_of_coset[coset];
    const u64* in = a.in + (size_t)blockIdx.y * a.in_batch_stride + (size_t)col * a.in_col_stride + (a.in_coset_blocks ? (size_t)blk * n : 0);
    u64* out = a.out + (size_t)blockIdx.y * a.out_batch_stride + (size_t)col * a.out_col_stride + (size_t)blk * n;
    const u64* pre = a.pre ? a.pre + (size_t)coset * n : nullptr;
    const u64* post = a.post ? a.post + (size_t)coset * n : nullptr;
    for (u32 i = threadIdx.x; i < n; i += blockDim.x) {
        u64 v = in[i];
        u32 dst = a.bitrev_in ? (__brev(i) >> (32 - logn)) : i;
        if (pre) v = gl::mul_nb(v, pre[dst]);
        lds[dst] = v;
    }
    __syncthreads();
    const int tw_shift = a.log_nmax - logn;
    int s = logn - 1;
    if (logn & 1) {
        const u32 h = 1u << s;
        for (u32 t = threadIdx.x; t < (n >> 1); t += blockDim.x) {
            u32 pos = t & (h - 1);
            u32 i = ((t >> s) << (s + 1)) | pos;
            u64 x = lds[i], y = lds[i + h];
            u64 w = a.tw[(size_t)(pos << (logn - 1 - s)) << tw_shift];
            lds[i] = gl::add(x, y);
            lds[i + h] = gl::mul_nb(gl::sub(x, y), w);
        }
        __syncthreads();
        s--;
    }
    for (; s >= 1; s -= 2) {
        const u32 h = 1u << s, q = h >> 1;
        for (u32 t = threadIdx.x; t < (n >> 2); t += blockDim.x) {
            u32 pos = t & (q - 1);
            u32 i = ((t >> (s - 1)) << (s + 1)) | pos;
            u64 a0 = lds[i], a1 = lds[i + q], a2 = lds[i + h], a3 = lds[i + h + q];
            u64 w0 = a.tw[(size_t)(pos << (logn - 1 - s)) << tw_shift];
            u64 w1 = a.tw[(size_t)((pos + q) << (logn - 1 - s)) << tw_shift];
            u64 b0 = gl::add(a0, a2), b2 = gl::mul_nb(gl::sub(a0, a2), w0);
            u64 b1 = gl::add(a1, a3), b3 = gl::mul_nb(gl::sub(a1, a3), w1);
            u64 w2 = a.tw[(size_t)(pos << (logn - s)) << tw_shift];
            lds[i] = gl::add(b0, b1);
            lds[i + q] = gl::mul_nb(gl::sub(b0, b1), w2);
            lds[i + h] = gl::add(b2, b3);
            lds[i + h + q] = gl::mul_nb(gl::sub(b2, b3), w2);
        }
        __syncthreads();
    }
    for (u32 i = threadIdx.x; i < n; i += blockDim.x) {
        u32 src = a.bitrev_out ? (__brev(i) >> (32 - logn)) : i;
        u64 v = lds[src];
        if (post)
            v = gl::mul_nb(v, post[i]);
        else if (a.post_scalar != 1)
            v = gl::mul_nb(v, a.post_scalar);
        out[i] = v;
    }
}

__device__ __forceinline__ u32 ntt_pad(u32 i) { return i + (i >> 4); }
struct NttLdsWalk {
    u32 a0, step;
    __device__ __forceinline__ NttLdsWalk(u32 base, u32 stride) : a0(8 * ntt_pad(base)), step(stride >= 16 ? 8 * (stride + (stride >> 4)) : 8 * stride) {}
    __device__ __forceinline__ u64& at(u64* lds, int r) const { return *(u64*)((char*)lds + (a0 + (u32)r * step)); }
};
__device__ __forceinline__ void ntt_r16_load_tw(u64* w, const u64* __restrict__ tw, u32 tp, int m, int tw_log, int nstages) {
#pragma unroll
    for (int A = 0; A < 4; A++) {
        if (A >= nstages) break;
        const int half = 8 >> A, base = 16 - 2 * half, sh = tw_log - (m + 4 - A);
        const u32 off0 = tp << (sh + 3), dj = 1u << (m + sh + 3);
#pragma unroll
        for (int j = 0; j < 8; j++)
            if (j < half) w[base + j] = *(const u64*)((const char*)tw + (off0 + (u32)j * dj));
    }
}
template <int A>
__device__ __forceinline__ void ntt_r16_stage(u64* x, const u64* w) {
    constexpr int half = 8 >> A, base = 16 - 2 * half;
#pragma unroll
    for (int r = 0; r < 16; r++) {
        if (r & half) continue;
        const u64 u = x[r], v = x[r + half];
        x[r] = gl::add(u, v);
        x[r + half] = gl::mul_nb(gl::sub(u, v), w[base + r % half]);
    }
}
template <int A>
__device__ __forceinline__ void ntt_r16_stage_m0(u64* x, const u64* w) {
    constexpr int half = 8 >> A, base = 16 - 2 * half;
#pragma unroll
    for (int r = 0; r < 16; r++) {
        if (r & half) continue;
        const u64 u = x[r], v = x[r + half];
        x[r] = gl::add(u, v);
        x[r + half] = (r % half) ? gl::mul_nb(gl::sub(u, v), w[base + r % half]) : gl::sub(u, v);
    }
}
__device__ __forceinline__ void wave_lds_sync() {
    __builtin_amdgcn_fence(__ATOMIC_RELEASE, "wavefront");
    __builtin_amdgcn_wave_barrier();
    __builtin_amdgcn_fence(__ATOMIC_ACQUIRE, "wavefront");
}
__device__ __forceinline__ u32 xcd_swizzle(u32 b, u32 grid) { return (grid & 7) ? b : (b & 7) * (grid >> 3) + (b >> 3); }
__device__ __forceinline__ void loads_issued() { asm volatile("" ::: "memory"); }
template <bool SPLIT>
__global__ __launch_bounds__(1024) void k_ntt_r16(NttArgs a) {
    extern __shared__ __align__(16) u64 lds[];
    const int logn = SPLIT ? a.logn - 1 : a.logn;
    const u32 n = 1u << logn, T = n >> 4, t = threadIdx.x;
    const u32 bid = xcd_swizzle(blockIdx.x, gridDim.x);
    const u32 unit = SPLIT ? bid >> 1 : bid, half = SPLIT ? (bid & 1) : 0;
    const u32 col = unit / a.cosets, coset = unit % a.cosets;
    const u32 blk = a.block_of_coset[coset];
    const size_t full = (size_t)1 << a.logn;
    const u64* in = a.in + (size_t)blockIdx.y * a.in_batch_stride + (size_t)col * a.in_col_stride + (a.in_coset_blocks ? (size_t)blk * full : 0);
    u64* out = a.out + (size_t)blockIdx.y * a.out_batch_stride + (size_t)col * a.out_col_stride + (size_t)blk * full + (size_t)half * n;
    const u64* pre = a.pre ? a.pre + (size_t)coset * full : nullptr;
    const u64* post = a.post ? a.post + (size_t)coset * full : nullptr;
    u64 x[16];
    u64 w[15];
    bool tw_in_flight = false;
    if (SPLIT) {
        if (pre) {
            const u64 S = pre[n];
            const u64* scale = half ? (a.pre_tw ? a.pre_tw + (size_t)coset * n : nullptr) : pre;
            if (!half || scale) {
                u64 uu[16], vv[16], sc[16];
#pragma unroll
                for (int k = 0; k < 16; k++) uu[k] = in[t + T * k];
#pragma unroll
                for (int k = 0; k < 16; k++) vv[k] = in[t + T * k + n];
#pragma unroll
                for (int k = 0; k < 8; k++) sc[k] = scale[t + T * k];
                loads_issued();
#pragma unroll
                for (int k = 0; k < 16; k++) {
                    if (k == 4) {
                        loads_issued();
#pragma unroll
                        for (int j = 8; j < 16; j++) sc[j] = scale[t + T * j];
                        loads_issued();
                    }
                    if (k == 12) {
                        loads_issued();
                        ntt_r16_load_tw(w, a.tw, t, logn - 4, a.log_nmax, 4);
                        loads_issued();
                    }
                    const u64 v = gl::mul_nb(vv[k], S);
                    x[k] = gl::mul_nb(half ? gl::sub(uu[k], v) : gl::add(uu[k], v), sc[k]);
                }
                tw_in_flight = true;
            } else {
#pragma unroll
                for (int k = 0; k < 16; k++) {
                    const u32 i = t + T * k;
                    const u64 u = in[i], v = gl::mul_nb(in[i + n], S);
                    x[k] = gl::mul_nb(gl::mul_nb(gl::sub(u, v), pre[i]), a.tw[(size_t)i << (a.log_nmax - a.logn)]);
                }
            }
        } else {
#pragma unroll
            for (int k = 0; k < 16; k++) {
                const u32 i = t + T * k;
                const u64 u = in[i], v = in[i + n];
                x[k] = half ? gl::mul_nb(gl::sub(u, v), a.tw[(size_t)i << (a.log_nmax - a.logn)]) : gl::add(u, v);
            }
        }
    } else if (a.bitrev_in) {
#pragma unroll
        for (int k = 0; k < 16; k++) {
            const u32 i = t + T * k, dst = __brev(i) >> (32 - logn);
            u64 v = in[i];
            if (pre) v = gl::mul_nb(v, pre[dst]);
            lds[ntt_pad(dst)] = v;
        }
        __syncthreads();
        {
            const NttLdsWalk w0(t, T);
#pragma unroll
            for (int k = 0; k < 16; k++) x[k] = w0.at(lds, k);
        }
    } else {
#pragma unroll
        for (int k = 0; k < 16; k++) x[k] = in[t + T * k];
        const int rem0 = (logn & 3) ? (logn & 3) : 4;
        if (pre) {
            u64 pv[16];
#pragma unroll
            for (int k = 0; k < 16; k++) pv[k] = pre[t + T * k];
            loads_issued();
#pragma unroll
            for (int k = 0; k < 16; k++) {
                if (k == 8) {
                    loads_issued();
                    ntt_r16_load_tw(w, a.tw, t, logn - 4, a.log_nmax, rem0);
                    loads_issued();
                }
                x[k] = gl::mul_nb(x[k], pv[k]);
            }
        } else {
            ntt_r16_load_tw(w, a.tw, t, logn - 4, a.log_nmax, rem0);
            loads_issued();
        }
        tw_in_flight = true;
    }
    if (SPLIT) {
        if (!tw_in_flight) ntt_r16_load_tw(w, a.tw, t, logn - 4, a.log_nmax, 4);
        ntt_r16_stage<0>(x, w);
        ntt_r16_stage<1>(x, w);
        ntt_r16_stage<2>(x, w);
        ntt_r16_stage<3>(x, w);
        int logN = logn - 4;
        const int rem = (logN & 3) ? (logN & 3) : 4;
        int m = logN - 4;
        u32 tp = t & ((1u << m) - 1);
        ntt_r16_load_tw(w, a.tw, tp, m, a.log_nmax, rem);
        {
            const NttLdsWalk wr(t, T);
#pragma unroll
            for (int r = 0; r < 16; r++) wr.at(lds, r) = x[r];
        }
        __syncthreads();
        u32 base_idx = ((t >> m) << logN) | tp, stride = 1u << m;
        {
            const NttLdsWalk rd(base_idx, stride);
#pragma unroll
            for (int r = 0; r < 16; r++) x[r] = rd.at(lds, r);
        }
        ntt_r16_stage<0>(x, w);
        if (rem >= 2) ntt_r16_stage<1>(x, w);
        if (rem >= 3) ntt_r16_stage<2>(x, w);
        if (rem >= 4) ntt_r16_stage<3>(x, w);
        for (logN -= rem; logN >= 4; logN -= 4) {
            m = logN - 4;
            tp = t & ((1u << m) - 1);
            ntt_r16_load_tw(w, a.tw, tp, m, a.log_nmax, 4);
            {
                const NttLdsWalk wr(base_idx, stride);
#pragma unroll
                for (int r = 0; r < 16; r++) wr.at(lds, r) = x[r];
            }
            wave_lds_sync();
            base_idx = ((t >> m) << logN) | tp;
            stride = 1u << m;
            {
                const NttLdsWalk rd(base_idx, stride);
#pragma unroll
                for (int r = 0; r < 16; r++) x[r] = rd.at(lds, r);
            }
            if (m == 0) {
                ntt_r16_stage_m0<0>(x, w);
                ntt_r16_stage_m0<1>(x, w);
                ntt_r16_stage_m0<2>(x, w);
                ntt_r16_stage_m0<3>(x, w);
            } else {
                ntt_r16_stage<0>(x, w);
                ntt_r16_stage<1>(x, w);
                ntt_r16_stage<2>(x, w);
                ntt_r16_stage<3>(x, w);
            }
        }
        {
            const NttLdsWalk wr(base_idx, stride);
#pragma unroll
            for (int r = 0; r < 16; r++) wr.at(lds, r) = x[r];
        }
        wave_lds_sync();
        const u32 first = ((t >> 6) << 10) | (t & 63);
        const NttLdsWalk fin(first, 64);
#pragma unroll
        for (int k = 0; k < 16; k++) {
            u64 v = fin.at(lds, k);
            if (a.post_scalar != 1) v = gl::mul_nb(v, a.post_scalar);
            out[first + 64 * k] = v;
        }
        return;
    }
    const int rem = (logn & 3) ? (logn & 3) : 4;
    if (!tw_in_flight) ntt_r16_load_tw(w, a.tw, t, logn - 4, a.log_nmax, rem);
    ntt_r16_stage<0>(x, w);
    if (rem >= 2) ntt_r16_stage<1>(x, w);
    if (rem >= 3) ntt_r16_stage<2>(x, w);
    if (rem >= 4) ntt_r16_stage<3>(x, w);
    u32 base_idx = t, stride = T;
    for (int logN = logn - rem; logN >= 4; logN -= 4) {
        const int m = logN - 4;
        const u32 tp = t & ((1u << m) - 1);
        ntt_r16_load_tw(w, a.tw, tp, m, a.log_nmax, 4);
        {
            const NttLdsWalk wr(base_idx, stride);
#pragma unroll
            for (int r = 0; r < 16; r++) wr.at(lds, r) = x[r];
        }
        __syncthreads();
        base_idx = ((t >> m) << logN) | tp;
        stride = 1u << m;
        {
            const NttLdsWalk rd(base_idx, stride);
#pragma unroll
            for (int r = 0; r < 16; r++) x[r] = rd.at(lds, r);
        }
        if (m == 0) {
            ntt_r16_stage_m0<0>(x, w);
            ntt_r16_stage_m0<1>(x, w);
            ntt_r16_stage_m0<2>(x, w);
            ntt_r16_stage_m0<3>(x, w);
        } else {
            ntt_r16_stage<0>(x, w);
            ntt_r16_stage<1>(x, w);
            ntt_r16_stage<2>(x, w);
            ntt_r16_stage<3>(x, w);
        }
    }
    {
        const NttLdsWalk wr(base_idx, stride);
#pragma unroll
        for (int r = 0; r < 16; r++) wr.at(lds, r) = x[r];
    }
    __syncthreads();
    const NttLdsWalk fin(t, T);
#pragma unroll
    for (int k = 0; k < 16; k++) {
        const u32 i = t + T * k;
        u64 v = (!SPLIT && a.bitrev_out) ? lds[ntt_pad(__brev(i) >> (32 - logn))] : fin.at(lds, k);
        if (post)
            v = gl::mul_nb(v, post[(size_t)half * n + i]);
        else if (a.post_scalar != 1)
            v = gl::mul_nb(v, a.post_scalar);
        out[i] = v;
    }
}


struct Pass1Args {
    const u64* in;
    u64* out;
    const u64* tw;
    const u64* pre;
    const u64* out_tw;
    size_t in_col_stride, out_col_stride, in_batch_stride, out_batch_stride;
    int logn, log_n1, log_T, cosets, in_coset_blocks, xcd_swizzle;
    u32 block_of_coset[8];
};
__device__ __forceinline__ void ntt_p1_load_tw(u64* w, const u64* __restrict__ tw, u32 tp, int m, int log_T, int tw_log, int nstages) {
#pragma unroll
    for (int A = 0; A < 4; A++) {
        if (A >= nstages) break;
        const int half = 8 >> A, base = 16 - 2 * half, q = m + 4 - A - log_T;
#pragma unroll
        for (int j = 0; j < 8; j++)
            if (j < half) w[base + j] = tw[(size_t)((tp + ((u32)j << m)) >> log_T) << (tw_log - q)];
    }
}
__global__ __launch_bounds__(256, 4) void k_ntt_pass1_r16(Pass1Args a) {
    extern __shared__ __align__(16) u64 lds[];
    const u32 T = 1u << a.log_T, t = threadIdx.x;
    const int log_n2 = a.logn - a.log_n1;
    const u32 n2 = 1u << log_n2, tiles = n2 >> a.log_T;
    const u32 bid = a.xcd_swizzle ? xcd_swizzle(blockIdx.x, gridDim.x) : blockIdx.x;
    const u32 tile = bid % tiles, cc = bid / tiles, col = cc / a.cosets, coset = cc % a.cosets;
    const u32 blk = a.block_of_coset[coset];
    const size_t n = (size_t)1 << a.logn;
    const u64* in = a.in + (size_t)blockIdx.y * a.in_batch_stride + (size_t)col * a.in_col_stride + (a.in_coset_blocks ? (size_t)blk * n : 0);
    u64* out = a.out + (size_t)blockIdx.y * a.out_batch_stride + (size_t)col * a.out_col_stride + (size_t)blk * n;
    const u64* pre = a.pre ? a.pre + (size_t)coset * n : nullptr;
    const u32 j2_0 = tile << a.log_T;
    u64 x[16], w[15];
    const int rem = (a.log_n1 & 3) ? (a.log_n1 & 3) : 4;
    const u32 at = (t >> a.log_T) * n2 + j2_0 + (t & (T - 1));
    auto step = [&](int k) -> u32 { return ((256u * (u32)k) >> a.log_T) * n2 + ((256u * (u32)k) & (T - 1)); };
#pragma unroll
    for (int k = 0; k < 16; k++) x[k] = in[at + step(k)];
    if (pre) {
        u64 pv[16];
#pragma unroll
        for (int k = 0; k < 16; k++) pv[k] = pre[at + step(k)];
        loads_issued();
#pragma unroll
        for (int k = 0; k < 16; k++) {
            if (k == 8) {
                loads_issued();
                ntt_p1_load_tw(w, a.tw, t, 8, a.log_T, a.logn, rem);
                loads_issued();
            }
            x[k] = gl::mul_nb(x[k], pv[k]);
        }
    } else {
        ntt_p1_load_tw(w, a.tw, t, 8, a.log_T, a.logn, rem);
        loads_issued();
    }
    ntt_r16_stage<0>(x, w);
    if (rem >= 2) ntt_r16_stage<1>(x, w);
    if (rem >= 3) ntt_r16_stage<2>(x, w);
    if (rem >= 4) ntt_r16_stage<3>(x, w);
    u32 base_idx = t, stride = 256;
    for (int logN = 12 - rem; logN - 4 >= a.log_T; logN -= 4) {
// ... 914 lines not shown
```

### plonky2-aes_amd/csrc/prover_gpu.hip

```cpp
#include <hip/hip_runtime.h>
#include <chrono>
#include <cstring>

#include <algorithm>
#include <map>
#include <memory>
#include <mutex>
#include <random>
#include <string>
#include <thread>

#include "capi_common.h"
#include "os_random.h"
#include "kernels.h"
#include "kernels2.h"
#include "kernels_compress.h"
#include "kernels_keccak.h"
#include "kernels_merkle.h"
#include "kernels_witness_io.h"
#include "merkle_host.h"
#include "verifier.h"

using namespace p2;
using namespace p2k;
// ... 186 lines not shown
        a.gate_kind[g] = c.gates[g];
        a.gate_sel[g] = c.selector_index[g];
        a.group_lo[g] = c.groups[c.selector_index[g]].first;
        a.group_hi[g] = c.groups[c.selector_index[g]].second;
    }
}

static int ecstep_gate_index(const Circuit& c) {
    for (size_t g = 0; g < c.gates.size(); g++)
        if (c.gates[g] == p2::G_ECSTEP) return (int)g;
    return -1;
}

static inline dim3 g1(size_t work, u32 block, u32 y = 1, u32 z = 1) { return dim3((u32)((work + block - 1) / block), y, z); }

static const u32 R16_MIN_BITS = 8;
static size_t r16_lds_bytes(int logn) { return 8 * (((size_t)1 << logn) + ((size_t)1 << (logn - 4))); }
static int run_ntt(Lane& L, const Domain& D, const char* name, NttArgs a, u32 cols, u32 batch) {
    a.log_nmax = (int)D.logn;
    if ((u32)a.logn >= 13 && !a.bitrev_in && !a.bitrev_out && !a.post) {
        LAUNCH(L, name, k_ntt_r16<true>, dim3(2 * cols * a.cosets, batch), dim3(1u << (a.logn - 5)), r16_lds_bytes(a.logn - 1), a);
        return 0;
    }
    if ((u32)a.logn >= R16_MIN_BITS) {
        LAUNCH(L, name, k_ntt_r16<false>, dim3(cols * a.cosets, batch), dim3(1u << (a.logn - 4)), r16_lds_bytes(a.logn), a);
        return 0;
    }
    size_t shmem = (size_t)8 << a.logn;
    LAUNCH(L, name, k_ntt_lds, dim3(cols * a.cosets, batch), dim3(1024), shmem, a);
    return 0;
}
static const u32 LDS_NTT_MAX_BITS = 14;
static hipError_t raise_ntt_lds_limits() {
    const std::pair<const void*, int> limits[] = {{(const void*)k_ntt_lds, 128 * 1024},
                                                  {(const void*)k_ntt_r16<false>, (int)r16_lds_bytes(LDS_NTT_MAX_BITS)},
                                                  {(const void*)k_ntt_r16<true>, (int)r16_lds_bytes(LDS_NTT_MAX_BITS - 1)},
                                                  {(const void*)k_ntt_pass1_r16, 64 * 1024}};
    for (const auto& l : limits)
        if (hipError_t e = hipFuncSetAttribute(l.first, hipFuncAttributeMaxDynamicSharedMemorySize, l.second)) return e;
    return hipSuccess;
}
static int ensure_pass1_table(Lane& L, Domain& D, Allocs& mem, const u64* tw_full, u32 logn) {
    if (logn <= LDS_NTT_MAX_BITS || D.pass1_out_tw.count(tw_full)) return 0;
    u64* t = nullptr;
    if (dalloc(mem, &t, (size_t)1 << logn)) return P2_ERR_HIP;
    hipLaunchKernelGGL(k_pass1_out_tw, g1((size_t)1 << logn, 256), dim3(256), 0, L.stream, tw_full, t, (int)logn, (int)(logn - 12));
    HIPCHECK(hipGetLastError());
    D.pass1_out_tw[tw_full] = t;
    return 0;
}
static int ntt_big(Lane& L, const Domain& D, const char* name, const u64* in, u64* out, const u64* tw_full, const u64* pre, u32 logn, u32 cols, u32 cosets,
                   const u32* block_of_coset, int in_coset_blocks, size_t in_col_stride, size_t out_col_stride, size_t in_batch_stride,
                   size_t out_batch_stride, u64 post_scalar, u32 batch) {
    const u32 log_n2 = 12, log_n1 = logn - log_n2;
    u32 log_T = 12 - log_n1;
    if (log_T < 2) return set_error("transform too large for the two-pass NTT"), P2_ERR_INVALID;
    Pass1Args a{};
    a.in = in;
    a.out = out;
    a.tw = tw_full;
    a.pre = pre;
    a.in_col_stride = in_col_stride;
    a.out_col_stride = out_col_stride;
    a.in_batch_stride = in_batch_stride;
    a.out_batch_stride = out_batch_stride;
    a.logn = (int)logn;
    a.log_n1 = (int)log_n1;
    a.log_T = (int)log_T;
    a.cosets = (int)cosets;
    a.in_coset_blocks = in_coset_blocks;
    for (u32 j = 0; j < 8; j++) a.block_of_coset[j] = block_of_coset ? block_of_coset[j] : 0;
    u32 tiles = (1u << log_n2) >> log_T;
    auto it = D.pass1_out_tw.find(tw_full);
    if (it == D.pass1_out_tw.end()) return set_error("internal: no pass-1 twiddle table for this transform"), P2_ERR_INVALID;
    a.out_tw = it->second;
    a.xcd_swizzle = (cosets > 1 && !in_coset_blocks) ? 1 : 0;
    const std::string name1 = std::string(name) + "_pass1";
    LAUNCH(L, name1, k_ntt_pass1_r16, dim3(tiles * cols * cosets, batch), dim3(256), r16_lds_bytes(12), a);
    if (out_col_stride != ((size_t)cosets << logn)) return set_error("internal: two-pass NTT needs densely packed output blocks"), P2_ERR_INVALID;
    NttArgs b{};
    b.in = out;
    b.out = out;
    b.tw = tw_full;
    b.post_scalar = post_scalar;
    b.in_col_stride = b.out_col_stride = (size_t)1 << log_n2;
    b.in_batch_stride = b.out_batch_stride = out_batch_stride;
    b.logn = (int)log_n2;
    b.log_nmax = (int)logn;
    b.cosets = 1;
    size_t rows = ((size_t)cols * cosets) << log_n1;
    LAUNCH(L, name, k_ntt_r16<false>, dim3((u32)rows, batch), dim3(1u << (log_n2 - 4)), r16_lds_bytes((int)log_n2), b);
    return 0;
}
static int build_transform_tables(Lane& L, Domain& D, Allocs& mem, u64** shift_inv_pows) {
    const size_t n = D.n();
    {
        std::vector<u64> sub(n), twi(n);
        u64 w = gl::root_of_unity((int)D.logn), wi = gl::inv(w), x = 1, xi = 1;
        for (size_t i = 0; i < n; i++) {
            sub[i] = x;
            twi[i] = xi;
            x = gl::mul(x, w);
            xi = gl::mul(xi, wi);
        }
        if (upload(mem, &D.d_tw_fwd_full, sub.data(), n)) return P2_ERR_HIP;
        if (upload(mem, &D.d_tw_inv_full, twi.data(), n)) return P2_ERR_HIP;
        D.d_tw_fwd = D.d_tw_fwd_full;
        D.d_tw_inv = D.d_tw_inv_full;
        if (ensure_pass1_table(L, D, mem, D.d_tw_fwd_full, D.logn) || ensure_pass1_table(L, D, mem, D.d_tw_inv_full, D.logn)) return P2_ERR_HIP;
        u32 logn_r = D.logn;
        for (u32 r = 0; r < D.arities.size(); r++) {
            logn_r -= D.arities[r];
            if (logn_r > LDS_NTT_MAX_BITS) {
                size_t n_r = (size_t)1 << logn_r;
                std::vector<u64> t(n_r);
                for (size_t i = 0; i < n_r; i++) t[i] = sub[i << (D.logn - logn_r)];
                if (upload(mem, &D.d_tw_fwd_round[r + 1], t.data(), n_r)) return P2_ERR_HIP;
                if (ensure_pass1_table(L, D, mem, D.d_tw_fwd_round[r + 1], logn_r)) return P2_ERR_HIP;
            }
        }
    }
    {
        u32 logn_r = D.logn;
        u64 shift = gl::MULT_GEN;
        for (u32 r = 0; r <= D.arities.size(); r++) {
            size_t n_r = (size_t)1 << logn_r;
            std::vector<u64> bases(8);
            u64 wl = gl::root_of_unity((int)(logn_r + D.rate_bits));
            for (u32 j = 0; j < 8; j++) bases[j] = gl::mul(shift, gl::pow(wl, j));
            u64* d_b;
            if (upload(mem, &d_b, bases.data(), 8)) return P2_ERR_HIP;
            if (dalloc(mem, &D.d_shift_pows[r], 8 * n_r)) return P2_ERR_HIP;
            hipLaunchKernelGGL(k_pow_table, g1(n_r, 256, 8), dim3(256), 0, L.stream, D.d_shift_pows[r], d_b, (u32)n_r, (u64)1);
            if (r == 0 && D.logn >= 13 && D.logn <= LDS_NTT_MAX_BITS) {
                if (dalloc(mem, &D.d_shift_tw, 8 * (n_r / 2))) return P2_ERR_HIP;
                hipLaunchKernelGGL(k_mul_tables, g1(n_r / 2, 256, 8), dim3(256), 0, L.stream, D.d_shift_tw, D.d_shift_pows[0], n_r, D.d_tw_fwd, 0, (u32)(n_r / 2));
            }
            if (r == 0 && shift_inv_pows) {
                std::vector<u64> ib(8);
                for (u32 j = 0; j < 8; j++) ib[j] = gl::inv(bases[j]);
                u64* d_ib;
                if (upload(mem, &d_ib, ib.data(), 8)) return P2_ERR_HIP;
                if (dalloc(mem, shift_inv_pows, 8 * n_r)) return P2_ERR_HIP;
                hipLaunchKernelGGL(k_pow_table, g1(n_r, 256, 8), dim3(256), 0, L.stream, *shift_inv_pows, d_ib, (u32)n_r, gl::inv((u64)n % gl::P));
            }
            if (r < D.arities.size()) {
                shift = gl::pow(shift, (u64)1 << D.arities[r]);
                logn_r -= D.arities[r];
            }
        }
        HIPCHECK(hipGetLastError());
    }
    return 0;
}
static int intt_cols(Lane& L, const Domain& D, const u64* vals, u64* coeffs, u32 cols, size_t batch_stride, u32 batch, u64* scratch = nullptr,
                     size_t scratch_batch_stride = 0) {
    const size_t n = D.n();
    if (D.logn > LDS_NTT_MAX_BITS) {
        if (!scratch) return set_error("internal: large iNTT needs scratch"), P2_ERR_INVALID;
        if (ntt_big(L, D, "intt", vals, scratch, D.d_tw_inv_full, nullptr, D.logn, cols, 1, nullptr, 0, n, n, batch_stride, scratch_batch_stride,
                    gl::inv((u64)n % gl::P), batch))
            return P2_ERR_HIP;
        LAUNCH(L, "bitrev_copy", k_bitrev_copy, g1(n, 256, batch, cols), dim3(256), 0, scratch, n, scratch_batch_stride, coeffs, n, batch_stride,
               (int)D.logn, 1u, (const u64*)nullptr, 0u);
        return 0;
    }
    NttArgs a{};
    a.in = vals;
    a.out = coeffs;
    a.tw = D.d_tw_inv;
    a.post_scalar = gl::inv((u64)n % gl::P);
    a.in_col_stride = a.out_col_stride = n;
    a.in_batch_stride = a.out_batch_stride = batch_stride;
    a.logn = (int)D.logn;
    a.cosets = 1;
    a.bitrev_out = 1;
    return run_ntt(L, D, "intt", a, cols, batch);
}
static int lde_cols(Lane& L, const Domain& D, const u64* coeffs, size_t in_batch_stride, u64* lde, size_t out_batch_stride, u32 cols, u32 round, u32 batch) {
    u32 logn_r = D.logn;
    for (u32 r = 0; r < round; r++) logn_r -= D.arities[r];
    u32 blocks[8];
    for (u32 j = 0; j < 8; j++) blocks[j] = gl::bitrev(j, (int)D.rate_bits);
    if (logn_r > LDS_NTT_MAX_BITS) {
        if (round != 0 && D.d_tw_fwd_round[round] == nullptr) return set_error("internal: missing round twiddles"), P2_ERR_INVALID;
        const u64* tw = round == 0 ? D.d_tw_fwd_full : D.d_tw_fwd_round[round];
        return ntt_big(L, D, "lde", coeffs, lde, tw, D.d_shift_pows[round], logn_r, cols, 8, blocks, 0, (size_t)1 << logn_r, (size_t)8 << logn_r,
                       in_batch_stride, out_batch_stride, 1, batch);
    }
    NttArgs a{};
    a.in = coeffs;
    a.out = lde;
    a.tw = D.d_tw_fwd;
    a.pre = D.d_shift_pows[round];
    a.pre_tw = round == 0 ? D.d_shift_tw : nullptr;
    a.post_scalar = 1;
    a.in_col_stride = (size_t)1 << logn_r;
    a.out_col_stride = (size_t)8 << logn_r;
    a.in_batch_stride = in_batch_stride;
    a.out_batch_stride = out_batch_stride;
    a.logn = (int)logn_r;
    a.cosets = 1 << D.rate_bits;
    for (u32 j = 0; j < 8; j++) a.block_of_coset[j] = blocks[j];
    return run_ntt(L, D, "lde", a, cols, batch);
}
static int quotient_chunks(Lane& L, const Domain& D, u64* qvals, u64* qres, u64* coef, u32 chunks, size_t coef_batch_stride, u32 B, const u64* shift_inv_pows,
                           const u64* w8inv, const u64* qscale) {
    const size_t n = D.n(), N = n << D.rate_bits, qs = (size_t)chunks * N;
    if (D.logn > LDS_NTT_MAX_BITS) {
        u32 ident[8] = {0, 1, 2, 3, 4, 5, 6, 7};
        LAUNCH(L, "bitrev_copy", k_bitrev_copy, g1(n, 256, B, chunks * 8), dim3(256), 0, qvals, N, qs, qres, N, qs, (int)D.logn, 8u, (const u64*)nullptr, 0u);
        if (ntt_big(L, D, "quotient_intt", qres, qvals, D.d_tw_inv_full, nullptr, D.logn, chunks, 8, ident, 1, N, N, qs, qs, 1, B)) return P2_ERR_HIP;
        LAUNCH(L, "bitrev_copy", k_bitrev_copy, g1(n, 256, B, chunks * 8), dim3(256), 0, qvals, N, qs, qres, N, qs, (int)D.logn, 8u, shift_inv_pows, 1u);
    } else {
        NttArgs t{};
        t.in = qvals;
        t.out = qres;
        t.tw = D.d_tw_inv;
        t.post = shift_inv_pows;
        t.post_scalar = 1;
        t.in_col_stride = t.out_col_stride = N;
        t.in_batch_stride = t.out_batch_stride = qs;
        t.logn = (int)D.logn;
        t.cosets = 8;
        t.bitrev_in = 1;
        t.bitrev_out = 1;
        t.in_coset_blocks = 1;
        for (u32 j = 0; j < 8; j++) t.block_of_coset[j] = gl::bitrev(j, 3);
        if (run_ntt(L, D, "quotient_intt", t, chunks, B)) return P2_ERR_HIP;
    }
    LAUNCH(L, "quotient_chunks", k_quotient_chunks_rev, g1(n, 256, B, chunks), dim3(256), 0, qres, coef, (u32)n, qs, coef_batch_stride, w8inv, qscale);
    return 0;
}
static void quotient_chunk_scales(u32 logn, u64* w8inv, u64* qscale) {
    const u64 gn = gl::pow(gl::MULT_GEN, (u64)1 << logn), w8 = gl::root_of_unity(3);
    for (u32 j = 0; j < 8; j++) {
        w8inv[j] = gl::inv(gl::pow(w8, j));
        qscale[j] = gl::mul(gl::inv(gl::pow(gn, j)), gl::inv(8));
    }
}
struct TreeKernels {
    decltype(&k_hash_leaves) leaves;
    decltype(&k_hash_fri_leaves) fri_leaves;
    decltype(&k_merkle_level) level;
    bool fused_top;
};
static TreeKernels tree_kernels(u32 hasher) {
    if (hasher == HASHER_KECCAK) return {k_kc_leaves, k_kc_fri_leaves, k_kc_level, false};
    return {k_hash_leaves, k_hash_fri_leaves, k_merkle_level, true};
}
static int merkle_levels(Lane& L, const Domain& D, Tree& t, u32 batch) {
    const u32 cap_h = D.cap_height;
    if (t.bits <= cap_h) return 0;
    const u32 levels = t.bits - cap_h;
    const TreeKernels k = tree_kernels(D.hasher);
    const u32 fused = k.fused_top && batch <= 16 ? std::min<u32>(levels, 9) : 0;
    const u32 top_threads = 256;
    for (u32 l = 0; l < levels - fused; l++) {
        size_t parents = ((size_t)1 << t.bits) >> (l + 1);
        LAUNCH(L, "merkle_level", k.level, g1(parents, 256, batch), dim3(256), 0, t.dig + level_off(t.bits, l), t.dig + level_off(t.bits, l + 1), parents, t.stride());
    }
    if (fused) {
        const u32 direct = fused > 6 ? fused - 6 : 0;
        if (direct) LAUNCH(L, "merkle_top", k_merkle_top, dim3(1u << cap_h, batch), dim3(top_threads), 0, t.dig, t.stride(), t.bits, levels - fused, direct);
        LAUNCH(L, "merkle_top", k_merkle_top_coop, dim3(1u << cap_h, batch), dim3(256), 0, t.dig, t.stride(), t.bits, levels - fused + direct, fused - direct);
    }
    return 0;
}
static int merkle_build(Lane& L, const Domain& D, const u64* data, u32 cols, u32 active, size_t col_stride, size_t batch_stride, Tree& t, u32 batch) {
    size_t leaves = (size_t)1 << t.bits;
    LAUNCH(L, "hash_leaves", tree_kernels(D.hasher).leaves, g1(leaves, 256, batch), dim3(256), 0, data, (int)cols, (int)active, col_stride, batch_stride, leaves, t.dig,
           t.stride());
    return merkle_levels(L, D, t, batch);
}
static int challenger(p2_circuit* C, Workspace& W, u32 stage, const u64* observe, size_t stride, u32 len, u32 aux, u64 mod, u32 batch) {
    ChalArgs a{};
    a.st = W.d_chal_state;
    a.chal = W.d_chal;
    a.observe = observe;
    a.observe_stride = stride;
    a.observe_len = len;
    a.batch = batch;
    a.stage = stage;
    a.aux = aux;
    a.mod = mod;
    a.digest = C->d_digest;
    a.pi_hash = C->c.pi_slots.empty() ? nullptr : W.d_pi_hash;
    a.status = W.d_status;
    LAUNCH(W.lane, "challenger", k_challenger, g1((size_t)batch * 16, 64), dim3(64), 0, a);
    return 0;
}

static int circuit_setup(p2_circuit* C) {
    const Circuit& c = C->c;
    Domain& D = C->dom;
    const size_t n = C->n, N = C->N;
    const u32 R = c.cfg.num_routed_wires, ncc = c.num_constants_cols(), np = c.num_preprocessed();
    if (c.cfg.num_challenges > 2) return set_error("k_perm_chunks handles at most two challenges"), P2_ERR_INVALID;
    if (c.num_partial_products() + 1 > PERM_MAX_CHUNKS) return set_error("more partial-product chunks than k_perm_scan holds in registers"), P2_ERR_INVALID;
    {
        WitnessSchedule ws = schedule_witness(c, std::min<u32>(C->opt_witness_fuse, WITNESS_KMAX));
// ... 1906 lines not shown
                acc_dot2_k(ka, kb, v, ua, ub);
                wka = gl::add_ref(wka, M(v, ua));
                wkb = gl::add_ref(wkb, M(v, ub));
            }
            if (acc_value(ka) != wka || acc_value(kb) != wkb) b++;
        }
        {
            const u64 l0 = rnd(), l1 = rnd(), h0 = rnd_uniform(), h1 = rnd_uniform(), h1w = rnd_uniform();
            const E2 got = tabpow_mul(gl::e2(l0, l1), h0, h1, h1w);
            if (got.a != gl::add_ref(M(l0, h0), M(l1, h1w)) || got.b != gl::add_ref(M(l0, h1), M(l1, h0))) b++;
            const u64 c = rnd_uniform() % gl::P, d = rnd_uniform() % gl::P;
            const E2 lo = gl::e2(l0 % gl::P, l1 % gl::P), want = gl::mul(lo, gl::e2(c, d)), have = tabpow_mul(lo, c, d, gl::mul(d, gl::W_EXT));
            if (have.a != want.a || have.b != want.b) b++;
        }
        {
            const u64 dA = rnd_uniform() % gl::P, dB = rnd_uniform() % gl::P, dAl = rnd_uniform() % gl::P, dD = rnd_uniform() % gl::P;
            u64 cur = rnd(), tsum = rnd(), tprod = rnd(), lsum = rnd(), lprod = rnd();
            u64 rcur = cur % gl::P, rtsum = tsum % gl::P, rtprod = tprod % gl::P, rlsum = lsum % gl::P, rlprod = lprod % gl::P;
            for (int st = 0; st < 3; st++) {
                const u64 win = rnd() % gl::P, wout = rnd() % gl::P, wm = rnd() % gl::P;
                const u64 f = gl::sub_ref(dAl, gl::add_ref(gl::mul_ref(dA, wout), win));
                const u64 ncur = gl::add_ref(gl::mul_ref(rcur, dD), gl::add_ref(gl::mul_ref(dB, wout), win));
                const u64 nts = gl::add_ref(gl::mul_ref(rtsum, f), gl::mul_ref(wm, rtprod)), ntp = gl::mul_ref(rtprod, f);
                const u64 nls = gl::add_ref(gl::mul_ref(rlsum, f), rlprod), nlp = gl::mul_ref(rlprod, f);
                {
                    u64 c2 = rcur, s2 = rtsum, p2_ = rtprod;
                    lut_step<false>(c2, s2, p2_, dA, dB, dAl, dD, win, wout, wm);
                    if (c2 != ncur || s2 != nts || p2_ != ntp) b++;
                }
                lut_step<true>(cur, tsum, tprod, dA, dB, dAl, dD, win, wout, wm);
                lu_step(lsum, lprod, dA, dAl, win, wout);
                rcur = ncur, rtsum = nts, rtprod = ntp, rlsum = nls, rlprod = nlp;
                if (glf::canon(cur) != rcur || glf::canon(tsum) != rtsum || glf::canon(tprod) != rtprod) b++;
                if (lsum != rlsum || lprod != rlprod) b++;
            }
            const u64 diff = rnd() % gl::P;
            if (glf::canon(lut_close<true>(tprod, tsum, diff)) != gl::sub_ref(gl::mul_ref(rtprod, diff), rtsum)) b++;
            if (glf::canon(lu_close(lprod, lsum, diff)) != gl::add_ref(gl::mul_ref(rlprod, diff), rlsum)) b++;
            if (gl::sub(dAl, glf::canon(cur)) != gl::sub_ref(dAl, rcur)) b++;
        }
        {
            const u64 a = rnd(), c = rnd() % gl::P;
            if (glf::canon(gl::sub(a, c)) != gl::sub_ref(a % gl::P, c)) b++;
            if (glf::canon(gl::add(a, c)) != gl::add_ref(a % gl::P, c) || glf::canon(gl::add(c, a)) != gl::add_ref(a % gl::P, c)) b++;
            if (glf::canon(gl::mul_nc(gl::sub(a, c), f0)) != M(gl::sub_ref(a % gl::P, c), f0)) b++;
        }
    }
    {
        const u64 one_nc = gl::P + 1 + (x & 0), top = ~0ull - (x & 0);
        if (glf::canon(gl::sub(0, one_nc)) == gl::sub_ref(0, one_nc % gl::P)) b++;
        if (glf::canon(gl::add(top, top)) == gl::add_ref(top % gl::P, top % gl::P)) b++;
    }
    if (b) atomicAdd(bad, b);
}
}

int p2_selftest_lazy_device(uint64_t seed, size_t threads, int device) {
    if (hipSetDevice(device) != hipSuccess) return set_error("no such HIP device"), -P2_ERR_HIP;
    if (threads == 0 || threads > ((size_t)1 << 30)) return set_error("thread count out of range"), -P2_ERR_INVALID;
    Allocs mem;
    unsigned long long* d = nullptr;
    if (dalloc(mem, &d, 1) || hipMemset(d, 0, 8) != hipSuccess) return set_error("hipMalloc failed"), -P2_ERR_HIP;
    hipLaunchKernelGGL(p2k::k_selftest_lazy, dim3((u32)((threads + 255) / 256)), dim3(256), 0, 0, d, (u64)seed, threads);
    unsigned long long h = 0;
    if (hipError_t e = hipMemcpy(&h, d, 8, hipMemcpyDeviceToHost)) return set_error(hipGetErrorString(e)), -P2_ERR_HIP;
    return (int)std::min<unsigned long long>(h, 0x7FFFFFFF);
}
namespace p2k {
__device__ __forceinline__ void borrow_pair(u64 r, u64& pw, u64& q) {
    const int j = 33 + 3 * (int)((r >> 56) % 11);
    const u64 m = 1 + (r & 0xFFFFFFFFFFFFull) % (((u64)1 << (j - 32)) - 1);
    pw = (u64)1 << j;
    q = m << (96 - j);
}
__device__ void ref_r16_stage(u64* x, const u64* w, int A) {
    const int half = 8 >> A, base = 16 - 2 * half;
    for (int r = 0; r < 16; r++) {
        if (r & half) continue;
        const u64 u = x[r], v = x[r + half];
        x[r] = gl::add_ref(u, v);
        x[r + half] = gl::mul_ref(gl::sub_ref(u, v), w[base + r % half]);
    }
}
__global__ void k_selftest_ntt(unsigned long long* bad, u64 seed, size_t threads) {
    const size_t t = (size_t)blockIdx.x * blockDim.x + threadIdx.x;
    if (t >= threads) return;
    u64 x = (seed | 1) + 0x9E3779B97F4A7C15ull * (t + 1);
    auto step = [&]() {
        x ^= x << 13;
        x ^= x >> 7;
        x ^= x << 17;
        return x;
    };
    auto rnd = [&]() {
        const u64 r = step();
        return lazy_draw(r, (u32)(r >> 40));
    };
    auto C = [](u64 v) { return v >= gl::P ? v - gl::P : v; };
    auto rndc = [&]() { return C(rnd()); };
    auto M = [&](u64 a, u64 b) { return gl::mul_ref(C(a), C(b)); };
    const bool odd = t & 1;
    unsigned long long b = 0;
    for (int i = 0; i < 16; i++) {
        {
            const u64 a = rnd(), c = rnd();
            if (gl::mul_nb(a, c) != M(a, c)) b++;
        }
        u64 pw, q;
        borrow_pair(step(), pw, q);
        {
            const u64 ea = odd ? step() : pw, eb = odd ? step() : q, want = M(ea, eb);
            if (gl::mul_nb(ea, eb) != want || gl::mul_nb(eb, ea) != want) b++;
        }
        {
            const u64 u = rndc(), v = rndc(), w = rndc();
            if (gl::add(u, v) != gl::add_ref(u, v)) b++;
            if (gl::mul_nb(gl::sub(u, v), w) != gl::mul_ref(gl::sub_ref(u, v), w)) b++;
            const u64 ub = gl::add_ref(v, q), wb = odd ? w : pw;
            if (gl::add(ub, v) != gl::add_ref(ub, v)) b++;
            if (gl::mul_nb(gl::sub(ub, v), wb) != gl::mul_ref(q, wb)) b++;
        }
        u64 xs[16], tw[15], got[16], want[16];
        for (int k = 0; k < 16; k++) xs[k] = rndc();
        for (int k = 0; k < 15; k++) tw[k] = rndc();
        if (!odd) {
            const int r = i & 7;
            tw[r] = pw;
            xs[r] = gl::add_ref(xs[r + 8], q);
        }
        for (int k = 0; k < 16; k++) got[k] = want[k] = xs[k];
        ntt_r16_stage<0>(got, tw);
        ntt_r16_stage<1>(got, tw);
        ntt_r16_stage<2>(got, tw);
        ntt_r16_stage<3>(got, tw);
        for (int A = 0; A < 4; A++) ref_r16_stage(want, tw, A);
        for (int k = 0; k < 16; k++) b += got[k] != want[k];
        tw[0] = tw[8] = tw[12] = tw[14] = 1;
        for (int k = 0; k < 16; k++) got[k] = want[k] = xs[k];
        ntt_r16_stage_m0<0>(got, tw);
        ntt_r16_stage_m0<1>(got, tw);
        ntt_r16_stage_m0<2>(got, tw);
        ntt_r16_stage_m0<3>(got, tw);
        for (int A = 0; A < 4; A++) ref_r16_stage(want, tw, A);
        for (int k = 0; k < 16; k++) b += got[k] != want[k];
        for (int k = 0; k < 16; k++) got[k] = xs[k];
        ntt_r16_stage<0>(got, tw);
        ntt_r16_stage<1>(got, tw);
        ntt_r16_stage<2>(got, tw);
        ntt_r16_stage<3>(got, tw);
        for (int k = 0; k < 16; k++) b += got[k] != want[k];
        {
            const int A = 1 + i % 3, half = 8 >> A, base = 16 - 2 * half, r = ((i >> 2) & 1) * 2 * half + (i % half);
            for (int k = 0; k < 16; k++) got[k] = want[k];
            if (!odd) {
                tw[base + r % half] = pw;
                got[r] = gl::add_ref(got[r + half], q);
            }
            for (int k = 0; k < 16; k++) want[k] = got[k];
            if (A == 1) ntt_r16_stage<1>(got, tw);
            if (A == 2) ntt_r16_stage<2>(got, tw);
            if (A == 3) ntt_r16_stage<3>(got, tw);
            ref_r16_stage(want, tw, A);
            for (int k = 0; k < 16; k++) b += got[k] != want[k];
        }
    }
    {
        const u64 one_nc = gl::P + 1 + (x & 0), w = (u64)1 << 33;
        if (gl::mul_nb(gl::sub(0, one_nc), w) == gl::mul_ref(gl::sub_ref(0, C(one_nc)), w)) b++;
    }
    if (b) atomicAdd(bad, b);
}
}

int p2_selftest_ntt_device(uint64_t seed, size_t threads, int device) {
    if (hipSetDevice(device) != hipSuccess) return set_error("no such HIP device"), -P2_ERR_HIP;
    if (threads == 0 || threads > ((size_t)1 << 30)) return set_error("thread count out of range"), -P2_ERR_INVALID;
    Allocs mem;
    unsigned long long* d = nullptr;
    if (dalloc(mem, &d, 1) || hipMemset(d, 0, 8) != hipSuccess) return set_error("hipMalloc failed"), -P2_ERR_HIP;
    hipLaunchKernelGGL(p2k::k_selftest_ntt, dim3((u32)((threads + 255) / 256)), dim3(256), 0, 0, d, (u64)seed, threads);
    unsigned long long h = 0;
    if (hipError_t e = hipMemcpy(&h, d, 8, hipMemcpyDeviceToHost)) return set_error(hipGetErrorString(e)), -P2_ERR_HIP;
    return (int)std::min<unsigned long long>(h, 0x7FFFFFFF);
}
int p2_gpu_zeta_pows(const uint64_t* z, size_t n, uint64_t* pows, int device) {
    if (n == 0 || n > ((size_t)1 << 22) || (n & (n - 1))) return set_error("n must be a power of two up to 2^22"), P2_ERR_INVALID;
    if (z[0] >= gl::P || z[1] >= gl::P) return set_error("z is not canonical"), P2_ERR_INVALID;
    if (int rc = pick_device(device)) return rc;
    int logn = 0;
    while (((size_t)1 << logn) < n) logn++;
    std::vector<u64> chal(CH_WORDS, 0);
    chal[CH_ZETA] = z[0];
    chal[CH_ZETA + 1] = z[1];
    Allocs mem;
    u64 *d_chal, *d_tab, *d_pows;
    if (upload(mem, &d_chal, chal.data(), chal.size()) || dalloc(mem, &d_tab, 4 * zeta_tab_words((u32)n)) || dalloc(mem, &d_pows, 8 * n)) return P2_ERR_HIP;
    hipLaunchKernelGGL(k_zeta_tabs, g1(ZT_LO + zeta_tab_hi((u32)n), 256, 1, 4), dim3(256), 0, 0, d_chal, d_tab, (u32)n, gl::root_of_unity(logn));
    HIPCHECK(hipGetLastError());
    hipLaunchKernelGGL(k_zeta_pows, g1(n, 256, 1, 4), dim3(256), 0, 0, d_tab, d_pows, (size_t)8 * n, (u32)n);
    HIPCHECK(hipGetLastError());
    HIPCHECK(hipMemcpy(pows, d_pows, 8 * n * 8, hipMemcpyDeviceToHost));
    return P2_OK;
}

int p2_gpu_poseidon(uint64_t* states, size_t n_perm, int device) {
    if (int rc = pick_device(device)) return rc;
    Allocs mem;
    u64* d;
    if (upload(mem, &d, (const u64*)states, n_perm * 12)) return P2_ERR_HIP;
    hipLaunchKernelGGL(k_poseidon_states, g1(n_perm, 256), dim3(256), 0, 0, d, n_perm);
    HIPCHECK(hipGetLastError());
    HIPCHECK(hipMemcpy(states, d, n_perm * 96, hipMemcpyDeviceToHost));
    return P2_OK;
}
int p2_gpu_hash_leaves(const uint64_t* data, size_t cols, size_t active_cols, size_t num_leaves, size_t batch, uint64_t* digests, int device) {
    if (cols == 0 || cols > (1u << 20) || num_leaves == 0 || batch == 0 || batch > 65535) return set_error("shape out of range"), P2_ERR_INVALID;
    if (int rc = pick_device(device)) return rc;
    const size_t stored = std::min(active_cols, cols), in_words = std::max<size_t>(stored, 1) * num_leaves;
    Allocs mem;
    u64 *d_in, *d_out;
    if (dalloc(mem, &d_in, batch * in_words) || dalloc(mem, &d_out, batch * num_leaves * 4)) return P2_ERR_HIP;
    HIPCHECK(hipMemcpy(d_in, data, batch * stored * num_leaves * 8, hipMemcpyHostToDevice));
    hipLaunchKernelGGL(k_hash_leaves, g1(num_leaves, 256, (u32)batch), dim3(256), 0, 0, d_in, (int)cols, (int)active_cols, num_leaves, stored * num_leaves, num_leaves,
                       d_out, num_leaves * 4);
    HIPCHECK(hipGetLastError());
    HIPCHECK(hipMemcpy(digests, d_out, batch * num_leaves * 32, hipMemcpyDeviceToHost));
    return P2_OK;
}
int p2_gpu_partial_rounds(uint64_t* states, size_t count, int device) {
    if (count == 0 || count > (1u << 24)) return set_error("count out of range"), P2_ERR_INVALID;
    if (int rc = pick_device(device)) return rc;
    Allocs mem;
    u64* d;
    if (upload(mem, &d, (const u64*)states, count * 12)) return P2_ERR_HIP;
    hipLaunchKernelGGL(k_partial_rounds, g1(count, 256), dim3(256), 0, 0, d, count);
    HIPCHECK(hipGetLastError());
    HIPCHECK(hipMemcpy(states, d, count * 96, hipMemcpyDeviceToHost));
    return P2_OK;
}
int p2_gpu_ecstep_constraints(const uint64_t* wires, size_t count, uint64_t* out, int device) {
    if (count == 0 || count > (1u << 20) || !wires || !out) return set_error("count out of range"), P2_ERR_INVALID;
    for (size_t i = 0; i < 80 * count; i++)
        if (wires[i] >= gl::P) return set_error("p2_gpu_ecstep_constraints: non-canonical wire"), P2_ERR_INVALID;
    if (int rc = pick_device(device)) return rc;
    Allocs mem;
    u64 *d_in, *d_out;
    if (upload(mem, &d_in, (const u64*)wires, count * 80) || dalloc(mem, &d_out, count * 40)) return P2_ERR_HIP;
    hipLaunchKernelGGL(k_ecstep_selftest, g1(count, 256), dim3(256), 0, 0, d_in, count, d_out);
    HIPCHECK(hipGetLastError());
    HIPCHECK(hipMemcpy(out, d_out, count * 40 * 8, hipMemcpyDeviceToHost));
    return P2_OK;
}
int p2_gpu_merged_middle(uint64_t* states, size_t count, int device) {
    if (count == 0 || count > (1u << 24)) return set_error("count out of range"), P2_ERR_INVALID;
    if (int rc = pick_device(device)) return rc;
    Allocs mem;
    u64* d;
    if (upload(mem, &d, (const u64*)states, count * 12)) return P2_ERR_HIP;
    hipLaunchKernelGGL(k_merged_middle, g1(count, 256), dim3(256), 0, 0, d, count);
    HIPCHECK(hipGetLastError());
    HIPCHECK(hipMemcpy(states, d, count * 96, hipMemcpyDeviceToHost));
    return P2_OK;
}
int p2_gpu_merkle_level(const uint64_t* child, size_t num_parents, size_t batch, uint64_t* parent, int device) {
    if (num_parents == 0 || batch == 0 || batch > 65535) return set_error("shape out of range"), P2_ERR_INVALID;
    if (int rc = pick_device(device)) return rc;
// ... 351 lines not shown
```

Baseline: 775.0.

## Replace last radix-16 NTT stage twiddle multiplies with shift-based power-of-two reductions

In the final radix-16 step of the register NTT (m==0), the twiddles are powers of the 16th root of unity, which equals 2^12 in Goldilocks. The change swaps the general field multiplies there for specialised mul_pow2 shift-and-reduce routines, with a separate template path for the inverse transform selected by a new tw_inverse flag. It also adds branch-free sub and fused sub-multiply helpers that replace sub+mul pairs in butterflies, and a new red_tail_nb reduction. It peels the last stage out of the loop and adds selftests plus a host check that the root is 2^12. The aim is fewer 64-bit multiplies and fewer branches in NTT butterflies; in exchange the code grows and relies on the twiddle-table root assumption.

```diff
diff --git a/bindings/plonky2-hip/src/ffi.rs b/bindings/plonky2-hip/src/ffi.rs
--- a/bindings/plonky2-hip/src/ffi.rs
+++ b/bindings/plonky2-hip/src/ffi.rs
@@ -130,6 +130,9 @@
     pub fn p2_selftest_device(seed: u64, threads: usize, device: c_int) -> c_int;
     pub fn p2_selftest_lazy_device(seed: u64, threads: usize, device: c_int) -> c_int;
     pub fn p2_selftest_ntt_device(seed: u64, threads: usize, device: c_int) -> c_int;
+    pub fn p2_selftest_ntt_chain_device(n: usize, mismatches: *mut u64) -> c_int;
+    pub fn p2_host_mul_pow2(k: c_int, x: *const u64, count: usize, out: *mut u64) -> c_int;
+    pub fn p2_host_ntt_m0_shift(stage: c_int, j: c_int, inverse: c_int) -> c_int;
     pub fn p2_host_poseidon_known(states: *mut u64, n_perm: usize, kind: c_int, rows: u32, parts: c_int) -> c_int;
     pub fn p2_host_partial_rounds(states: *mut u64, count: usize) -> c_int;
     pub fn p2_host_merged_middle(states: *mut u64, count: usize) -> c_int;
diff --git a/include/p2aes.h b/include/p2aes.h
--- a/include/p2aes.h
+++ b/include/p2aes.h
@@ -161,6 +161,9 @@
 int p2_selftest_device(uint64_t seed, size_t threads, int device);
 int p2_selftest_lazy_device(uint64_t seed, size_t threads, int device);
 int p2_selftest_ntt_device(uint64_t seed, size_t threads, int device);
+int p2_selftest_ntt_chain_device(size_t n, uint64_t* mismatches);
+int p2_host_mul_pow2(int k, const uint64_t* x, size_t count, uint64_t* out);
+int p2_host_ntt_m0_shift(int stage, int j, int inverse);
 int p2_host_poseidon_known(uint64_t* states, size_t n_perm, int kind, uint32_t rows, int parts);
 int p2_host_partial_rounds(uint64_t* states, size_t count);
 int p2_host_merged_middle(uint64_t* states, size_t count);
diff --git a/plonky2-aes_amd/api.py b/plonky2-aes_amd/api.py
--- a/plonky2-aes_amd/api.py
+++ b/plonky2-aes_amd/api.py
@@ -212,6 +212,8 @@
         "p2_selftest_host": (C.c_int, [u64, sz, sz]), "p2_selftest_device": (C.c_int, [u64, sz, C.c_int]),
         "p2_selftest_lazy_device": (C.c_int, [u64, sz, C.c_int]),
         "p2_selftest_ntt_device": (C.c_int, [u64, sz, C.c_int]),
+        "p2_selftest_ntt_chain_device": (C.c_int, [sz, u64p]),
+        "p2_host_mul_pow2": (C.c_int, [C.c_int, u64p, sz, u64p]), "p2_host_ntt_m0_shift": (C.c_int, [C.c_int, C.c_int, C.c_int]),
         "p2_native_gf_2_8_mul": (C.c_uint8, [C.c_uint8, C.c_uint8]),
         "p2_native_aes_key_expansion": (None, [C.c_char_p, C.c_int, C.c_int, C.c_char_p]),
         "p2_native_aes_encrypt_block": (None, [C.c_char_p, C.c_int, C.c_int, C.c_char_p, C.c_char_p]),
diff --git a/plonky2-aes_amd/csrc/capi_host.cpp b/plonky2-aes_amd/csrc/capi_host.cpp
--- a/plonky2-aes_amd/csrc/capi_host.cpp
+++ b/plonky2-aes_amd/csrc/capi_host.cpp
@@ -637,6 +637,24 @@
     return (int)std::min<size_t>(bad, 0x7FFFFFFF);
 }
 
+int p2_host_mul_pow2(int k, const uint64_t* x, size_t count, uint64_t* out) {
+    if (count && (!x || !out)) return set_error("p2_host_mul_pow2: null argument"), P2_ERR_INVALID;
+    for (size_t i = 0; i < count; i++)
+        if (x[i] >= gl::P) return set_error("p2_host_mul_pow2: non-canonical operand"), P2_ERR_INVALID;
+    switch (k) {
+#define P2_POW2_CASE(K) \
+    case K: \
+        for (size_t i = 0; i < count; i++) out[i] = gl::mul_pow2<K>(x[i]); \
+        return P2_OK;
+        P2_POW2_CASE(12) P2_POW2_CASE(24) P2_POW2_CASE(36) P2_POW2_CASE(48) P2_POW2_CASE(60) P2_POW2_CASE(72) P2_POW2_CASE(84)
+#undef P2_POW2_CASE
+    }
+    return set_error("p2_host_mul_pow2: k must be a multiple of 12 in 12..84"), P2_ERR_INVALID;
+}
+int p2_host_ntt_m0_shift(int stage, int j, int inverse) {
+    if (stage < 0 || stage > 3 || j <= 0 || j >= (8 >> stage)) return -P2_ERR_INVALID;
+    return gl::ntt_m0_shift(stage, j, inverse != 0);
+}
 int p2_host_poseidon_known(uint64_t* states, size_t n_perm, int kind, uint32_t rows, int parts) {
     if (kind < 0 || kind > (int)glf::FR_ZERO_RATE || rows == 0 || rows > glf::ROWS_ALL) return set_error("kind must be 0..2 and rows a mask of words 0..11"), P2_ERR_INVALID;
     for (size_t i = 0; i < n_perm; i++) {
diff --git a/plonky2-aes_amd/csrc/gl.h b/plonky2-aes_amd/csrc/gl.h
--- a/plonky2-aes_amd/csrc/gl.h
+++ b/plonky2-aes_amd/csrc/gl.h
@@ -128,15 +128,12 @@
     asm("s_nop 1\n\tv_cndmask_b32_e64 %0, 0, 1, %1" : "=v"(r) : "s"(m));
     return r;
 }
-template <bool BRANCH = true>
+GL_D u32 ones_where_salu(sg m) {
+    u32 r;
+    asm("v_cndmask_b32_e64 %0, 0, -1, %1" : "=v"(r) : "s"(m));
+    return r;
+}
 GL_D u64 red_fix(u64 Rs, sg C, sg B) {
-    if (!BRANCH) {
-        const u32 dh = ones_where(B & ~C);
-        const u32 dl = ones_where(C & ~B) - dh;
-        u64 d = ((u64)dh << 32) | dl;
-        asm("" : "+v"(d));
-        return Rs + d;
-    }
     sg Cm = C;
     if (__builtin_expect(B != 0, 0)) {
         const u32 dh = ones_where(B & ~C);
@@ -160,6 +157,21 @@
         : "=&v"(lo), "=&v"(hi)
         : "v"((u32)yes), "v"((u32)no), "v"((u32)(yes >> 32)), "v"((u32)(no >> 32)), "s"(m));
     return ((u64)hi << 32) | lo;
+}
+GL_D u64 red_tail_nb(u64 lo, u64 H, sg k) {
+    sg C, b1_, B;
+    const u64 R = mad_eps_co((u32)H, lo, C);
+    u32 r0, r1;
+    asm("v_subb_co_u32_e64 %[r0], %[b1], %[Rl], %[Hh], %[k]\n\t"
+        "s_nop 1\n\t"
+        "v_subb_co_u32_e64 %[r1], %[B], %[Rh], 0, %[b1]"
+        : [r0] "=&v"(r0), [r1] "=&v"(r1), [b1] "=&s"(b1_), [B] "=&s"(B)
+        : [Rl] "v"((u32)R), [Rh] "v"((u32)(R >> 32)), [Hh] "v"((u32)(H >> 32)), [k] "s"(k));
+    const u32 dh = ones_where_salu(B & ~C);
+    const u32 dl = ones_where_salu(C & ~B) - dh;
+    u64 d = ((u64)dh << 32) | dl;
+    asm("" : "+v"(d));
+    return (((u64)r1 << 32) | r0) + d;
 }
 template <bool HAS_ADDEND, bool A_UNIFORM = false, bool BRANCH = true>
 GL_D u64 mulr_add_dev(u64 a, u64 b, u64 c) {
@@ -171,10 +183,11 @@
     Y = A_UNIFORM ? mad_co_k(a1, b0, Y, k) : mad_co(a1, b0, Y, k);
     const u64 H = (u64)a1 * b1 + (Y >> 32);
     const u64 lo = (Y << 32) | (u32)P;
+    if (!BRANCH) return red_tail_nb(lo, H, k);
     const u64 R = mad_eps_co((u32)H, lo, C);
     const u32 r0 = subb_co_settled((u32)R, (u32)(H >> 32), k, b1_);
     const u32 r1 = subb0_co((u32)(R >> 32), b1_, B);
-    return red_fix<BRANCH>(((u64)r1 << 32) | r0, C, B);
+    return red_fix(((u64)r1 << 32) | r0, C, B);
 }
 GL_D u64 red128_dev(u64 hi, u64 lo) {
     sg C, b1_, B;
@@ -266,6 +279,42 @@
     return mul_ref(a, b);
 #endif
 }
+GL_HD u64 sub_nb(u64 u, u64 v) {
+#if defined(__HIP_DEVICE_COMPILE__)
+    u32 d0, d1, e, dl;
+    sg b0, B;
+    asm("v_sub_co_u32_e64 %[d0], %[b0], %[ul], %[vl]\n\t"
+        "s_nop 1\n\t"
+        "v_subb_co_u32_e64 %[d1], %[B], %[uh], %[vh], %[b0]\n\t"
+        "s_nop 1\n\t"
+        "v_cndmask_b32_e64 %[e], 0, -1, %[B]\n\t"
+        "v_sub_u32_e32 %[dl], 0, %[e]"
+        : [d0] "=&v"(d0), [d1] "=&v"(d1), [e] "=&v"(e), [dl] "=&v"(dl), [b0] "=&s"(b0), [B] "=&s"(B)
+        : [ul] "v"((u32)u), [vl] "v"((u32)v), [uh] "v"((u32)(u >> 32)), [vh] "v"((u32)(v >> 32)));
+    u64 fix = ((u64)e << 32) | dl;
+    asm("" : "+v"(fix));
+    return (((u64)d1 << 32) | d0) + fix;
+#else
+    return sub_ref(u, v);
+#endif
+}
+GL_HD u64 sub_mul_nb(u64 u, u64 v, u64 w) { return mul_nb(sub_nb(u, v), w); }
+GL_HD u64 add_canon(u64 u, u64 v) { return add(u, v); }
+template <int K>
+GL_HD u64 mul_pow2(u64 x) {
+    static_assert(K > 0 && K < 96 && K != 64, "shift out of range");
+    if (K > 64) {
+        const u64 hi = x << ((K - 64) & 63), t = x >> ((128 - K) & 63);
+        return sub_nb((hi & EPS) * EPS, (t << 32) | (hi >> 32));
+    }
+    const u64 lo = x << (K & 63), hi = x >> ((64 - K) & 63);
+#if defined(__HIP_DEVICE_COMPILE__)
+    return canon_dev(red_tail_nb(lo, hi, 0));
+#else
+    return reduce128(hi, lo);
+#endif
+}
+constexpr int ntt_m0_shift(int A, int j, bool inverse) { return inverse ? 96 - 12 * (j << A) : 12 * (j << A); }
 GL_HD u64 sqr(u64 a) { return mul(a, a); }
 GL_HD u64 mul_add(u64 a, u64 b, u64 c) {
 #if defined(__HIP_DEVICE_COMPILE__)
diff --git a/plonky2-aes_amd/csrc/kernels.h b/plonky2-aes_amd/csrc/kernels.h
--- a/plonky2-aes_amd/csrc/kernels.h
+++ b/plonky2-aes_amd/csrc/kernels.h
@@ -1,5 +1,6 @@
 #pragma once
 #include <hip/hip_runtime.h>
+#include <utility>
 
 #include "circuit.h"
 #include "witness_schedule.h"
@@ -162,6 +163,7 @@
     const u64* in;
     u64* out;
     const u64* tw;
+    int tw_inverse;
     const u64* pre;
     const u64* pre_tw;
     const u64* post;
@@ -199,8 +201,8 @@
             u32 i = ((t >> s) << (s + 1)) | pos;
             u64 x = lds[i], y = lds[i + h];
             u64 w = a.tw[(size_t)(pos << (logn - 1 - s)) << tw_shift];
-            lds[i] = gl::add(x, y);
-            lds[i + h] = gl::mul_nb(gl::sub(x, y), w);
+            lds[i] = gl::add_canon(x, y);
+            lds[i + h] = gl::sub_mul_nb(x, y, w);
         }
         __syncthreads();
         s--;
@@ -213,13 +215,13 @@
             u64 a0 = lds[i], a1 = lds[i + q], a2 = lds[i + h], a3 = lds[i + h + q];
             u64 w0 = a.tw[(size_t)(pos << (logn - 1 - s)) << tw_shift];
             u64 w1 = a.tw[(size_t)((pos + q) << (logn - 1 - s)) << tw_shift];
-            u64 b0 = gl::add(a0, a2), b2 = gl::mul_nb(gl::sub(a0, a2), w0);
-            u64 b1 = gl::add(a1, a3), b3 = gl::mul_nb(gl::sub(a1, a3), w1);
+            u64 b0 = gl::add_canon(a0, a2), b2 = gl::sub_mul_nb(a0, a2, w0);
+            u64 b1 = gl::add_canon(a1, a3), b3 = gl::sub_mul_nb(a1, a3, w1);
             u64 w2 = a.tw[(size_t)(pos << (logn - s)) << tw_shift];
-            lds[i] = gl::add(b0, b1);
-            lds[i + q] = gl::mul_nb(gl::sub(b0, b1), w2);
-            lds[i + h] = gl::add(b2, b3);
-            lds[i + h + q] = gl::mul_nb(gl::sub(b2, b3), w2);
+            lds[i] = gl::add_canon(b0, b1);
+            lds[i + q] = gl::sub_mul_nb(b0, b1, w2);
+            lds[i + h] = gl::add_canon(b2, b3);
+            lds[i + h + q] = gl::sub_mul_nb(b2, b3, w2);
         }
         __syncthreads();
     }
@@ -258,20 +260,35 @@
     for (int r = 0; r < 16; r++) {
         if (r & half) continue;
         const u64 u = x[r], v = x[r + half];
-        x[r] = gl::add(u, v);
-        x[r + half] = gl::mul_nb(gl::sub(u, v), w[base + r % half]);
-    }
-}
-template <int A>
-__device__ __forceinline__ void ntt_r16_stage_m0(u64* x, const u64* w) {
-    constexpr int half = 8 >> A, base = 16 - 2 * half;
-#pragma unroll
-    for (int r = 0; r < 16; r++) {
-        if (r & half) continue;
-        const u64 u = x[r], v = x[r + half];
-        x[r] = gl::add(u, v);
-        x[r + half] = (r % half) ? gl::mul_nb(gl::sub(u, v), w[base + r % half]) : gl::sub(u, v);
-    }
+        x[r] = gl::add_canon(u, v);
+        x[r + half] = gl::sub_mul_nb(u, v, w[base + r % half]);
+    }
+}
+template <int A, bool INV, int R>
+__device__ __forceinline__ void ntt_r16_pair_m0(u64* x) {
+    constexpr int half = 8 >> A, j = R % half;
+    const u64 u = x[R], v = x[R + half];
+    x[R] = gl::add_canon(u, v);
+    if constexpr (j == 0)
+        x[R + half] = gl::sub_nb(u, v);
+    else
+        x[R + half] = gl::mul_pow2<gl::ntt_m0_shift(A, j, INV)>(INV ? gl::sub_nb(v, u) : gl::sub_nb(u, v));
+}
+template <int A, bool INV, int... Q>
+__device__ __forceinline__ void ntt_r16_stage_m0(u64* x, std::integer_sequence<int, Q...>) {
+    constexpr int half = 8 >> A;
+    (ntt_r16_pair_m0<A, INV, (Q / half) * 2 * half + Q % half>(x), ...);
+}
+template <int A, bool INV>
+__device__ __forceinline__ void ntt_r16_stage_m0(u64* x) {
+    ntt_r16_stage_m0<A, INV>(x, std::make_integer_sequence<int, 8>());
+}
+template <bool INV>
+__device__ __forceinline__ void ntt_r16_step_m0(u64* x) {
+    ntt_r16_stage_m0<0, INV>(x);
+    ntt_r16_stage_m0<1, INV>(x);
+    ntt_r16_stage_m0<2, INV>(x);
+    ntt_r16_stage_m0<3, INV>(x);
 }
 __device__ __forceinline__ void wave_lds_sync() {
     __builtin_amdgcn_fence(__ATOMIC_RELEASE, "wavefront");
@@ -324,7 +341,7 @@
                         loads_issued();
                     }
                     const u64 v = gl::mul_nb(vv[k], S);
-                    x[k] = gl::mul_nb(half ? gl::sub(uu[k], v) : gl::add(uu[k], v), sc[k]);
+                    x[k] = half ? gl::sub_mul_nb(uu[k], v, sc[k]) : gl::mul_nb(gl::add_canon(uu[k], v), sc[k]);
                 }
                 tw_in_flight = true;
             } else {
@@ -332,7 +349,7 @@
                 for (int k = 0; k < 16; k++) {
                     const u32 i = t + T * k;
                     const u64 u = in[i], v = gl::mul_nb(in[i + n], S);
-                    x[k] = gl::mul_nb(gl::mul_nb(gl::sub(u, v), pre[i]), a.tw[(size_t)i << (a.log_nmax - a.logn)]);
+                    x[k] = gl::mul_nb(gl::sub_mul_nb(u, v, pre[i]), a.tw[(size_t)i << (a.log_nmax - a.logn)]);
                 }
             }
         } else {
@@ -340,7 +357,7 @@
             for (int k = 0; k < 16; k++) {
                 const u32 i = t + T * k;
                 const u64 u = in[i], v = in[i + n];
-                x[k] = half ? gl::mul_nb(gl::sub(u, v), a.tw[(size_t)i << (a.log_nmax - a.logn)]) : gl::add(u, v);
+                x[k] = half ? gl::sub_mul_nb(u, v, a.tw[(size_t)i << (a.log_nmax - a.logn)]) : gl::add_canon(u, v);
             }
         }
     } else if (a.bitrev_in) {
@@ -408,35 +425,38 @@
         if (rem >= 2) ntt_r16_stage<1>(x, w);
         if (rem >= 3) ntt_r16_stage<2>(x, w);
         if (rem >= 4) ntt_r16_stage<3>(x, w);
-        for (logN -= rem; logN >= 4; logN -= 4) {
+        auto exchange = [&](int logN_next) {
+            const int m_next = logN_next - 4;
+            const u32 tp_next = t & ((1u << m_next) - 1);
+            {
+                const NttLdsWalk wr(base_idx, stride);
+#pragma unroll
+                for (int r = 0; r < 16; r++) wr.at(lds, r) = x[r];
+            }
+            wave_lds_sync();
+            base_idx = ((t >> m_next) << logN_next) | tp_next;
+            stride = 1u << m_next;
+            {
+                const NttLdsWalk rd(base_idx, stride);
+#pragma unroll
+                for (int r = 0; r < 16; r++) x[r] = rd.at(lds, r);
+            }
+        };
+        for (logN -= rem; logN > 4; logN -= 4) {
             m = logN - 4;
             tp = t & ((1u << m) - 1);
             ntt_r16_load_tw(w, a.tw, tp, m, a.log_nmax, 4);
-            {
-                const NttLdsWalk wr(base_idx, stride);
-#pragma unroll
-                for (int r = 0; r < 16; r++) wr.at(lds, r) = x[r];
-            }
-            wave_lds_sync();
-            base_idx = ((t >> m) << logN) | tp;
-            stride = 1u << m;
-            {
-                const NttLdsWalk rd(base_idx, stride);
-#pragma unroll
-                for (int r = 0; r < 16; r++) x[r] = rd.at(lds, r);
-            }
-            if (m == 0) {
-                ntt_r16_stage_m0<0>(x, w);
-                ntt_r16_stage_m0<1>(x, w);
-                ntt_r16_stage_m0<2>(x, w);
-                ntt_r16_stage_m0<3>(x, w);
-            } else {
-                ntt_r16_stage<0>(x, w);
-                ntt_r16_stage<1>(x, w);
-                ntt_r16_stage<2>(x, w);
-                ntt_r16_stage<3>(x, w);
-            }
-        }
+            exchange(logN);
+            ntt_r16_stage<0>(x, w);
+            ntt_r16_stage<1>(x, w);
+            ntt_r16_stage<2>(x, w);
+            ntt_r16_stage<3>(x, w);
+        }
+        exchange(4);
+        if (a.tw_inverse)
+            ntt_r16_step_m0<true>(x);
+        else
+            ntt_r16_step_m0<false>(x);
         {
             const NttLdsWalk wr(base_idx, stride);
 #pragma unroll
@@ -460,35 +480,37 @@
     if (rem >= 3) ntt_r16_stage<2>(x, w);
     if (rem >= 4) ntt_r16_stage<3>(x, w);
     u32 base_idx = t, stride = T;
-    for (int logN = logn - rem; logN >= 4; logN -= 4) {
-        const int m = logN - 4;
-        const u32 tp = t & ((1u << m) - 1);
-        ntt_r16_load_tw(w, a.tw, tp, m, a.log_nmax, 4);
+    auto exchange = [&](int logN_next) {
+        const int m_next = logN_next - 4;
+        const u32 tp_next = t & ((1u << m_next) - 1);
         {
             const NttLdsWalk wr(base_idx, stride);
 #pragma unroll
             for (int r = 0; r < 16; r++) wr.at(lds, r) = x[r];
         }
         __syncthreads();
-        base_idx = ((t >> m) << logN) | tp;
-        stride = 1u << m;
+        base_idx = ((t >> m_next) << logN_next) | tp_next;
+        stride = 1u << m_next;
         {
             const NttLdsWalk rd(base_idx, stride);
 #pragma unroll
             for (int r = 0; r < 16; r++) x[r] = rd.at(lds, r);
         }
-        if (m == 0) {
-            ntt_r16_stage_m0<0>(x, w);
-            ntt_r16_stage_m0<1>(x, w);
-            ntt_r16_stage_m0<2>(x, w);
-            ntt_r16_stage_m0<3>(x, w);
-        } else {
-            ntt_r16_stage<0>(x, w);
-            ntt_r16_stage<1>(x, w);
-            ntt_r16_stage<2>(x, w);
-            ntt_r16_stage<3>(x, w);
-        }
-    }
+    };
+    for (int logN = logn - rem; logN > 4; logN -= 4) {
+        const int m = logN - 4;
+        ntt_r16_load_tw(w, a.tw, t & ((1u << m) - 1), m, a.log_nmax, 4);
+        exchange(logN);
+        ntt_r16_stage<0>(x, w);
+        ntt_r16_stage<1>(x, w);
+        ntt_r16_stage<2>(x, w);
+        ntt_r16_stage<3>(x, w);
+    }
+    exchange(4);
+    if (a.tw_inverse)
+        ntt_r16_step_m0<true>(x);
+    else
+        ntt_r16_step_m0<false>(x);
     {
         const NttLdsWalk wr(base_idx, stride);
 #pragma unroll
diff --git a/plonky2-aes_amd/csrc/prover_gpu.hip b/plonky2-aes_amd/csrc/prover_gpu.hip
--- a/plonky2-aes_amd/csrc/prover_gpu.hip
+++ b/plonky2-aes_amd/csrc/prover_gpu.hip
@@ -292,6 +292,7 @@
     b.in = out;
     b.out = out;
     b.tw = tw_full;
+    b.tw_inverse = tw_full == D.d_tw_inv_full;
     b.post_scalar = post_scalar;
     b.in_col_stride = b.out_col_stride = (size_t)1 << log_n2;
     b.in_batch_stride = b.out_batch_stride = out_batch_stride;
@@ -307,6 +308,8 @@
     {
         std::vector<u64> sub(n), twi(n);
         u64 w = gl::root_of_unity((int)D.logn), wi = gl::inv(w), x = 1, xi = 1;
+        if (D.logn >= 4 && (gl::exp_pow2(w, (int)D.logn - 4) != ((u64)1 << 12) || gl::exp_pow2(wi, (int)D.logn - 4) != gl::inv((u64)1 << 12)))
+            return set_error("internal: the 16th root of unity of the twiddle tables is not 2^12"), P2_ERR_INVALID;
         for (size_t i = 0; i < n; i++) {
             sub[i] = x;
             twi[i] = xi;
@@ -379,6 +382,7 @@
     a.in = vals;
     a.out = coeffs;
     a.tw = D.d_tw_inv;
+    a.tw_inverse = 1;
     a.post_scalar = gl::inv((u64)n % gl::P);
     a.in_col_stride = a.out_col_stride = n;
     a.in_batch_stride = a.out_batch_stride = batch_stride;
@@ -427,6 +431,7 @@
         t.in = qvals;
         t.out = qres;
         t.tw = D.d_tw_inv;
+        t.tw_inverse = 1;
         t.post = shift_inv_pows;
         t.post_scalar = 1;
         t.in_col_stride = t.out_col_stride = N;
@@ -2499,6 +2504,17 @@
         x[r + half] = gl::mul_ref(gl::sub_ref(u, v), w[base + r % half]);
     }
 }
+__device__ void m0_twiddles(u64* tw, int inverse) {
+    const u64 w16 = inverse ? gl::P - (((u64)1 << 52) - ((u64)1 << 20)) : (u64)1 << 12;
+    for (int A = 0; A < 4; A++) {
+        const int half = 8 >> A, base = 16 - 2 * half;
+        for (int j = 0; j < half; j++) {
+            u64 v = 1;
+            for (int e = 0; e < (j << A); e++) v = gl::mul_ref(v, w16);
+            tw[base + j] = v;
+        }
+    }
+}
 __global__ void k_selftest_ntt(unsigned long long* bad, u64 seed, size_t threads) {
     const size_t t = (size_t)blockIdx.x * blockDim.x + threadIdx.x;
     if (t >= threads) return;
@@ -2552,14 +2568,16 @@
         ntt_r16_stage<3>(got, tw);
         for (int A = 0; A < 4; A++) ref_r16_stage(want, tw, A);
         for (int k = 0; k < 16; k++) b += got[k] != want[k];
-        tw[0] = tw[8] = tw[12] = tw[14] = 1;
-        for (int k = 0; k < 16; k++) got[k] = want[k] = xs[k];
-        ntt_r16_stage_m0<0>(got, tw);
-        ntt_r16_stage_m0<1>(got, tw);
-        ntt_r16_stage_m0<2>(got, tw);
-        ntt_r16_stage_m0<3>(got, tw);
-        for (int A = 0; A < 4; A++) ref_r16_stage(want, tw, A);
-        for (int k = 0; k < 16; k++) b += got[k] != want[k];
+        for (int inv = 0; inv < 2; inv++) {
+            m0_twiddles(tw, inv);
+            for (int k = 0; k < 16; k++) got[k] = want[k] = xs[k];
+            if (inv)
+                ntt_r16_step_m0<true>(got);
+            else
+                ntt_r16_step_m0<false>(got);
+            for (int A = 0; A < 4; A++) ref_r16_stage(want, tw, A);
+            for (int k = 0; k < 16; k++) b += got[k] != want[k];
+        }
         for (int k = 0; k < 16; k++) got[k] = xs[k];
         ntt_r16_stage<0>(got, tw);
         ntt_r16_stage<1>(got, tw);
@@ -2599,6 +2617,92 @@
     unsigned long long h = 0;
     if (hipError_t e = hipMemcpy(&h, d, 8, hipMemcpyDeviceToHost)) return set_error(hipGetErrorString(e)), -P2_ERR_HIP;
     return (int)std::min<unsigned long long>(h, 0x7FFFFFFF);
+}
+namespace p2k {
+__device__ __forceinline__ u64 chain_draw(u64 r, u32 sel) {
+    switch (sel % 12) {
+        case 0: return 0;
+        case 1: return 1;
+        case 2: return gl::P - 1;
+        case 3: return gl::EPS;
+        case 4: return (u64)1 << 32;
+        case 5: return gl::P - ((u64)1 << 32);
+        case 6: return ((r & 0xFFFF) | 1) << 48;
+        case 7: return (r & 0xFFFFFFFEull) << 32;
+        default: return r >= gl::P ? r - gl::P : r;
+    }
+}
+extern "C++" {
+template <int K>
+__device__ __forceinline__ u32 chain_check_pow2(u64 u, u64 v, u64 r, bool aimed) {
+    const u64 pw = K < 64 ? (u64)1 << (K & 63) : gl::mul_ref((u64)1 << 36, (u64)1 << ((K - 36) & 63));
+    u64 x = u;
+    if (aimed && K > 32) x = (1 + (r >> 8) % (((u64)1 << ((K - 32) & 63)) - 1)) << ((96 - K) & 63);
+    if (x >= gl::P) x = u;
+    u32 b = gl::mul_pow2<K>(x) != gl::mul_ref(x, pw);
+    b += gl::mul_pow2<K>(gl::sub_nb(v, u)) != gl::mul_ref(gl::sub_ref(u, v), gl::P - pw);
+    b += gl::mul_pow2<K>(gl::sub_nb(0, x)) != gl::mul_ref(x, gl::P - pw);
+    return b;
+}
+}
+__global__ void k_selftest_ntt_chain(unsigned long long* bad, size_t threads) {
+    const size_t t = (size_t)blockIdx.x * blockDim.x + threadIdx.x;
+    if (t >= threads) return;
+    u64 x = 0x2E77C4A1ull + 0x9E3779B97F4A7C15ull * (t + 1);
+    auto step = [&]() {
+        x ^= x << 13;
+        x ^= x >> 7;
+        x ^= x << 17;
+        return x;
+    };
+    auto rnd = [&]() {
+        const u64 r = step();
+        return chain_draw(r, (u32)(r >> 40));
+    };
+    const bool aimed = !(t & 1);
+    unsigned long long b = 0;
+    for (int i = 0; i < 64; i++) {
+        u64 u = rnd(), v = rnd(), w = rnd();
+        if ((t >> 1) & 1 && u < v) {
+            const u64 s = u;
+            u = v, v = s;
+        }
+        if (gl::sub_nb(u, v) != gl::sub_ref(u, v) || gl::add_canon(u, v) != gl::add_ref(u, v)) b++;
+        if (gl::sub_mul_nb(u, v, w) != gl::mul_ref(gl::sub_ref(u, v), w)) b++;
+        const u64 r = step();
+        if (aimed) {
+            u64 pw, q;
+            borrow_pair(r, pw, q);
+            const u64 ub = gl::add_ref(v, q);
+            if (gl::sub_mul_nb(ub, v, pw) != gl::mul_ref(q, pw)) b++;
+        } else {
+            if (gl::sub_mul_nb(v, u, r) != gl::mul_ref(gl::sub_ref(v, u), r >= gl::P ? r - gl::P : r)) b++;
+        }
+        b += chain_check_pow2<12>(u, v, r, aimed);
+        b += chain_check_pow2<24>(u, v, r, aimed);
+        b += chain_check_pow2<36>(u, v, r, aimed);
+        b += chain_check_pow2<48>(u, v, r, aimed);
+        b += chain_check_pow2<60>(u, v, r, aimed);
+        b += chain_check_pow2<72>(u, v, r, aimed);
+        b += chain_check_pow2<84>(u, v, r, aimed);
+    }
+    if (b) atomicAdd(bad, b);
+}
+}
+
+int p2_selftest_ntt_chain_device(size_t n, uint64_t* mismatches) {
+    if (!mismatches) return set_error("null argument"), P2_ERR_INVALID;
+    if (n == 0 || n > ((size_t)1 << 30)) return set_error("thread count out of range"), P2_ERR_INVALID;
+    if (int rc = pick_device(0)) return rc;
+    Allocs mem;
+    unsigned long long* d = nullptr;
+    if (dalloc(mem, &d, 1) || hipMemset(d, 0, 8) != hipSuccess) return set_error("hipMalloc failed"), P2_ERR_HIP;
+    hipLaunchKernelGGL(p2k::k_selftest_ntt_chain, dim3((u32)((n + 255) / 256)), dim3(256), 0, 0, d, n);
+    HIPCHECK(hipGetLastError());
+    unsigned long long h = 0;
+    HIPCHECK(hipMemcpy(&h, d, 8, hipMemcpyDeviceToHost));
+    *mismatches = h;
+    return P2_OK;
 }
 int p2_gpu_zeta_pows(const uint64_t* z, size_t n, uint64_t* pows, int device) {
     if (n == 0 || n > ((size_t)1 << 22) || (n & (n - 1))) return set_error("n must be a power of two up to 2^22"), P2_ERR_INVALID;
```

After: 778.3 (median of 6 runs). No clear change (+0.4%).
